# PeterFWS/Structure-PLP-SLAM

Measured on NVIDIA H100. Metric: frames_per_sec_extract_match_poseopt, higher is better.
Workload: dtype u8/f64

## Files before the change

### structure-plp-slam_b200/csrc/orb.cu

```cuda
#include "common.cuh"
#include <cuda.h>
#include <stdlib.h>
#include "brief_pattern.inc"

namespace plp {

namespace {

constexpr int kMaxLevels = 16;
constexpr int kPatchRadius = 19;
constexpr int kHalfPatch = 15;
constexpr int kCellSize = 64;
constexpr int kOverlap = 6;
constexpr int kCellCap = 1024;

struct LevelInfo {
    int w, h, pitch;
    size_t offset;
    size_t blur_offset;
    int cells_x, cells_y;
    int cell_base;
    int num_cells;
    int budget;
    int slot_base;
    int slot_cap;
    float scale_factor;
    float size;
};

struct CellDesc {
    short level, i, j, pad;
    short min_x, min_y, max_x, max_y;
};

struct BlurTile {
    short level, x0, y0, pad;
};

struct LevelKp {
    short x, y;
    int response;
};

struct OrbDev {
    int num_levels, rows, cols;
    int num_cells;
    int total_slots;
    int out_cap;
    int ini_thr, min_thr;
    LevelInfo lv[kMaxLevels];
    int u_max[16];
    const uint8_t *img0;
    size_t img0_step, img0_frame_stride;
    const uint8_t *mask;
    size_t mask_step;
    uint8_t *pyr;
    size_t pyr_frame_bytes;
    uint8_t *blur;
    size_t blur_frame_bytes;
    const BlurTile *blur_tiles;
    int num_blur_tiles;
    const CellDesc *cells;
    uint32_t *cell_buf;
    int *cell_cnt;
    LevelKp *lvl_kp;
    int *lvl_cnt;
    uint8_t *qt_scratch;
    size_t qt_scratch_per_job;
    int *status;
};

__device__ __forceinline__ const uint8_t *level_ptr(const OrbDev &P, int b, int l) {
    return l == 0 ? P.img0 + (size_t)b * P.img0_frame_stride : P.pyr + (size_t)b * P.pyr_frame_bytes + P.lv[l].offset;
}
__device__ __forceinline__ int level_pitch(const OrbDev &P, int l) { return l == 0 ? (int)P.img0_step : P.lv[l].pitch; }

constexpr int kBtW = 64, kBtH = 32;
constexpr int kBoxW = 96, kBoxH = kBtH + 6, kBoxX = 16;
static_assert(kBoxW >= kBoxX + kBtW + 3 && kBoxW % 16 == 0 && kBoxX % 16 == 0 && kBtW % 16 == 0,
              "TMA box: 16-byte aligned start and extent covering the 3-pixel halo");
static_assert(kBoxH % 2 == 0 && kBtH % 2 == 0, "the blur passes work on pairs of rows");
constexpr int kBoxStage = (kBoxH * kBoxW + 127) & ~127;
constexpr int kTilePitch = kBoxW;
constexpr int kTileRows = kCellSize + kOverlap;

struct BlurMaps {
    CUtensorMap m[kMaxLevels];
};

__device__ __forceinline__ uint32_t smem_u32(const void *p) { return (uint32_t)__cvta_generic_to_shared(p); }

__device__ __forceinline__ void mbar_init(uint32_t bar) { asm volatile("mbarrier.init.shared::cta.b64 [%0], 1;" ::"r"(bar)); }

__device__ __forceinline__ bool mbar_wait(uint32_t bar, uint32_t parity) {
    uint32_t done = 0;
    for (int spin = 0; spin < (1 << 14) && !done; ++spin)
        asm volatile(
            "{\n\t.reg .pred p;\n\tmbarrier.try_wait.parity.shared::cta.b64 p, [%1], %2;\n\tselp.u32 %0, 1, 0, p;\n\t}"
            : "=r"(done)
            : "r"(bar), "r"(parity)
            : "memory");
    return done != 0;
}

__device__ __forceinline__ void mbar_expect_tx(uint32_t bar, uint32_t bytes) {
    asm volatile("mbarrier.arrive.expect_tx.shared::cta.b64 _, [%0], %1;" ::"r"(bar), "r"(bytes) : "memory");
}

__device__ __forceinline__ void tma_box_load(uint32_t dst, const CUtensorMap *tm, int x, int y, int f, uint32_t bar) {
    asm volatile(
        "cp.async.bulk.tensor.3d.shared::cluster.global.mbarrier::complete_tx::bytes [%0], [%1, {%2, %3, %4}], [%5];"
        ::"r"(dst), "l"(tm), "r"(x), "r"(y), "r"(f), "r"(bar)
        : "memory");
}

constexpr int kResizeRows = 8;
__global__ void __launch_bounds__(256) pyr_resize_kernel(OrbDev P, int l, const short4 *__restrict__ xtab,
                                                         const short4 *__restrict__ ytab) {
    const int b = blockIdx.y;
    const int dw = P.lv[l].w, dh = P.lv[l].h, dpitch = P.lv[l].pitch;
    const int quads = (dw + 3) >> 2, strips = (dh + kResizeRows - 1) / kResizeRows;
    const int q = blockIdx.x * blockDim.x + threadIdx.x;
    if (q >= quads * strips) return;
    const int strip = q / quads, x0 = (q - strip * quads) * 4;
    const uint8_t *src = level_ptr(P, b, l - 1);
    const int spitch = level_pitch(P, l - 1);
    uint8_t *dst = const_cast<uint8_t *>(level_ptr(P, b, l));
    int sx0[4], sx1[4], a0[4], a1[4];
#pragma unroll
    for (int k = 0; k < 4; ++k) {
        const short4 xt = xtab[min(x0 + k, dw - 1)];
        sx0[k] = xt.x;
        sx1[k] = xt.y;
        a0[k] = xt.z;
        a1[k] = xt.w;
    }
    const int y_end = min(dh, (strip + 1) * kResizeRows);
    for (int y = strip * kResizeRows; y < y_end; ++y) {
        const short4 yt = ytab[y];
        const uint8_t *S0 = src + (size_t)yt.x * spitch, *S1 = src + (size_t)yt.y * spitch;
        const int b0 = yt.z, b1 = yt.w;
        uint32_t packed = 0;
#pragma unroll
        for (int k = 0; k < 4; ++k) {
            const int r0 = S0[sx0[k]] * a0[k] + S0[sx1[k]] * a1[k];
            const int r1 = S1[sx0[k]] * a0[k] + S1[sx1[k]] * a1[k];
            const int v = (((b0 * (r0 >> 4)) >> 16) + ((b1 * (r1 >> 4)) >> 16) + 2) >> 2;
            packed |= (uint32_t)(v & 0xff) << (8 * k);
        }
        *reinterpret_cast<uint32_t *>(dst + (size_t)y * dpitch + x0) = packed;
    }
}

__device__ __forceinline__ uint32_t fast_m_pair(const uint8_t *pa, const uint8_t *pb) {
    const uint32_t v2 = ((uint32_t)pa[0] + 256u) | (((uint32_t)pb[0] + 256u) << 16);
    uint32_t d[16];
#define PLP_RING(k, off) d[k] = v2 - ((uint32_t)pa[off] | ((uint32_t)pb[off] << 16))
    PLP_RING(0, 3 * kTilePitch);
    PLP_RING(1, 3 * kTilePitch + 1);
    PLP_RING(2, 2 * kTilePitch + 2);
    PLP_RING(3, 1 * kTilePitch + 3);
    PLP_RING(4, 3);
    PLP_RING(5, -1 * kTilePitch + 3);
    PLP_RING(6, -2 * kTilePitch + 2);
    PLP_RING(7, -3 * kTilePitch + 1);
    PLP_RING(8, -3 * kTilePitch);
    PLP_RING(9, -3 * kTilePitch - 1);
    PLP_RING(10, -2 * kTilePitch - 2);
    PLP_RING(11, -1 * kTilePitch - 3);
    PLP_RING(12, -3);
    PLP_RING(13, 1 * kTilePitch - 3);
    PLP_RING(14, 2 * kTilePitch - 2);
    PLP_RING(15, 3 * kTilePitch - 1);
#undef PLP_RING
    uint32_t e[16], d2[16], e2[16], d4[16], e4[16];
#pragma unroll
    for (int k = 0; k < 16; ++k) e[k] = 0x02000200u - d[k];
#pragma unroll
    for (int k = 0; k < 16; ++k) {
        d2[k] = __vimin3_s16x2(d[k], d[(k + 1) & 15], d[(k + 1) & 15]);
        e2[k] = __vimin3_s16x2(e[k], e[(k + 1) & 15], e[(k + 1) & 15]);
    }
#pragma unroll
    for (int k = 0; k < 16; ++k) {
        d4[k] = __vimin3_s16x2(d2[k], d2[(k + 2) & 15], d2[(k + 2) & 15]);
        e4[k] = __vimin3_s16x2(e2[k], e2[(k + 2) & 15], e2[(k + 2) & 15]);
    }
    uint32_t best = 0u;
#pragma unroll
    for (int k = 0; k < 16; ++k) {
        const uint32_t d9 = __vimin3_s16x2(d4[k], d4[(k + 4) & 15], d[(k + 8) & 15]);
        const uint32_t e9 = __vimin3_s16x2(e4[k], e4[(k + 4) & 15], e[(k + 8) & 15]);
        best = __vimax3_s16x2(best, d9, e9);
    }
    return best;
}

__device__ __forceinline__ bool masked(const OrbDev &P, unsigned y, unsigned x, float scale) {
    return P.mask[(size_t)(int)(y * scale) * P.mask_step + (int)(x * scale)] == 0;
}


constexpr int kTileX = kPatchRadius % 16;
constexpr int kTestX = kTileX + 3;
static_assert(kCellSize % 16 == 0 && kTestX % 4 == 2, "the pretests below form their words for tested x = 2 (mod 4)");
static_assert(kTileX + kCellSize + kOverlap <= kTilePitch, "a cell row fits a tile row");
constexpr int kFastBox2Row = kTileRows - kBoxH;
static_assert(kFastBox2Row > 0 && kFastBox2Row <= kBoxH && (kFastBox2Row * kTilePitch) % 128 == 0,
              "two boxes cover the tile rows; the second lands 128-byte aligned");
constexpr int kFastStage = (kTileRows * kTilePitch + 127) & ~127;
constexpr int kCornerWords = 4;
static_assert(kCornerWords * 32 >= kTilePitch + 32, "corner bitmap row");

#define PLP_TW(y, k) T32[(y) * (kTilePitch / 4) + (k)]

__device__ __forceinline__ uint32_t compass4(const uint32_t *T32, int y, int k, uint32_t t4) {
    const uint32_t c = __funnelshift_r(PLP_TW(y, k), PLP_TW(y, k + 1), 16);
    const uint32_t up = __funnelshift_r(PLP_TW(y - 3, k), PLP_TW(y - 3, k + 1), 16);
    const uint32_t dn = __funnelshift_r(PLP_TW(y + 3, k), PLP_TW(y + 3, k + 1), 16);
    const uint32_t lf = __funnelshift_r(PLP_TW(y, k - 1), PLP_TW(y, k), 24);
    const uint32_t rt = __funnelshift_r(PLP_TW(y, k + 1), PLP_TW(y, k + 2), 8);
    const uint32_t a0 = __vcmpgtu4(__vabsdiffu4(c, dn), t4), a4 = __vcmpgtu4(__vabsdiffu4(c, rt), t4);
    const uint32_t a8 = __vcmpgtu4(__vabsdiffu4(c, up), t4), a12 = __vcmpgtu4(__vabsdiffu4(c, lf), t4);
    const uint32_t sv = (a4 | a12) & (a0 | a8);
    const uint32_t m = sv & 0x01010101u;
    return (m | (m >> 7) | (m >> 14) | (m >> 21)) & 0xfu;
}

__device__ __forceinline__ uint32_t even8_4(const uint32_t *T32, int y, int k, uint32_t k7) {
    const uint32_t c = __funnelshift_r(PLP_TW(y, k), PLP_TW(y, k + 1), 16);
    auto gt = [&](uint32_t ring) -> uint32_t {
        const uint32_t d = __vabsdiffu4(c, ring);
        return (((d & 0x7f7f7f7fu) + k7) | d) & 0x80808080u;
    };
    const uint32_t e0 = gt(__funnelshift_r(PLP_TW(y + 3, k), PLP_TW(y + 3, k + 1), 16));
    const uint32_t e2 = gt(PLP_TW(y + 2, k + 1));
    const uint32_t e4 = gt(__funnelshift_r(PLP_TW(y, k + 1), PLP_TW(y, k + 2), 8));
    const uint32_t e6 = gt(PLP_TW(y - 2, k + 1));
    const uint32_t e8 = gt(__funnelshift_r(PLP_TW(y - 3, k), PLP_TW(y - 3, k + 1), 16));
    const uint32_t e10 = gt(PLP_TW(y - 2, k));
    const uint32_t e12 = gt(__funnelshift_r(PLP_TW(y, k - 1), PLP_TW(y, k), 24));
    const uint32_t e14 = gt(PLP_TW(y + 2, k));
    const uint32_t p0 = e0 & e2, p2 = e2 & e4, p4 = e4 & e6, p6 = e6 & e8, p8 = e8 & e10, p10 = e10 & e12, p12 = e12 & e14,
                   p14 = e14 & e0;
    const uint32_t r = (p0 & p4) | (p2 & p6) | (p4 & p8) | (p6 & p10) | (p8 & p12) | (p10 & p14) | (p12 & p0) | (p14 & p2);
    return ((r >> 7) | (r >> 14) | (r >> 21) | (r >> 28)) & 0xfu;
}
#undef PLP_TW

struct FastSmem {
    uint8_t score[kTileRows * kTilePitch];
    unsigned corner[kTileRows * kCornerWords];
    unsigned short list[kCellSize * kCellSize];
    unsigned rowbits[128];
    int rowbase[128];
    int wsum[4];
    int nsurv;
};

__device__ __forceinline__ void fast_smem_clear(FastSmem &S) {
    for (int i = threadIdx.x; i < kTileRows * kCornerWords; i += blockDim.x) S.corner[i] = 0u;
    if (threadIdx.x < 128) S.rowbits[threadIdx.x] = 0u;
    if (threadIdx.x == 0) S.nsurv = 0;
}

__device__ __forceinline__ void fast_cell_detect(const OrbDev &P, int ci, const uint8_t *tile, FastSmem &S) {
    const int tid = threadIdx.x, lane = tid & 31, warp = tid >> 5;
    const CellDesc cell = P.cells[ci];
    const int w = cell.max_x - cell.min_x, h = cell.max_y - cell.min_y;
    const float scale = P.lv[cell.level].scale_factor;
    bool skip = (w < 7 || h < 7);
    if (!skip && P.mask) {
        skip = masked(P, cell.min_y, cell.min_x, scale) || masked(P, cell.max_y, cell.min_x, scale) ||
               masked(P, cell.min_y, cell.max_x, scale) || masked(P, cell.max_y, cell.max_x, scale);
    }
    const int tw = w - 6, th = h - 6;
    const uint32_t *T32 = reinterpret_cast<const uint32_t *>(tile);
    for (int pass = 0; !skip; ++pass) {
        const int thr = pass == 0 ? P.ini_thr : P.min_thr;
        const uint32_t t4 = (uint32_t)min(thr, 255) * 0x01010101u;
        const bool strong = thr < 128;
        const uint32_t k7 = (uint32_t)(0x7f - min(thr, 127)) * 0x01010101u;
        for (int rp = warp; rp < (th + 1) / 2; rp += 8) {
            const int ry = 2 * rp + (lane >> 4), g = lane & 15;
            const int nv = tw - 4 * g;
            if (ry >= th || nv <= 0) continue;
            const int y = 3 + ry, k = (kTestX >> 2) + g;
            uint32_t nib = (strong ? even8_4(T32, y, k, k7) : compass4(T32, y, k, t4)) & (nv >= 4 ? 0xfu : (1u << nv) - 1u);
            if (!nib) continue;
            int pos = atomicAdd(&S.nsurv, __popc(nib));
            const int p0 = (y << 7) + kTestX + 4 * g;
            while (nib) {
                const int bit = __ffs(nib) - 1;
                nib &= nib - 1;
                S.list[pos++] = (unsigned short)(p0 + bit);
            }
        }
        __syncthreads();
        const int nsurv = S.nsurv;
        {
            const int half = (nsurv + 1) >> 1;
            for (int i = tid; i < half; i += 256) {
                const int pa = S.list[i];
                const bool has_b = i + half < nsurv;
                const int pb = has_b ? S.list[i + half] : pa;
                const int off_a = (pa >> 7) * kTilePitch + (pa & 127), off_b = (pb >> 7) * kTilePitch + (pb & 127);
                const uint32_t m2 = fast_m_pair(tile + off_a, tile + off_b);
                const int m_a = (int)(m2 & 0xffffu) - 256, m_b = (int)(m2 >> 16) - 256;
                if (m_a > thr) {
                    S.score[off_a] = (uint8_t)(m_a - 1);
                    atomicOr(&S.corner[(pa >> 7) * kCornerWords + ((pa & 127) >> 5)], 1u << (pa & 31));
                }
                if (has_b && m_b > thr) {
                    S.score[off_b] = (uint8_t)(m_b - 1);
                    atomicOr(&S.corner[(pb >> 7) * kCornerWords + ((pb & 127) >> 5)], 1u << (pb & 31));
                }
            }
        }
        __syncthreads();
        bool any_local = false;
        for (int i = tid; i < nsurv; i += 256) {
            const int p = S.list[i];
            const int y = p >> 7, x = p & 127;
            uint32_t nb[3];
#pragma unroll
            for (int r = 0; r < 3; ++r) {
                const unsigned *row = S.corner + (y - 1 + r) * kCornerWords + ((x - 1) >> 5);
                nb[r] = __funnelshift_r(row[0], row[1], (x - 1) & 31) & 7u;
            }
            if (!(nb[1] & 2u)) continue;
            const uint8_t *sp = S.score + y * kTilePitch + x;
            const int sc = sp[0];
            bool keep = true;
#pragma unroll
            for (int dy = -1; dy <= 1; ++dy)
#pragma unroll
                for (int dx = -1; dx <= 1; ++dx) {
                    if (dx == 0 && dy == 0) continue;
                    if (nb[dy + 1] & (1u << (dx + 1))) keep = keep && (sc > (int)sp[dy * kTilePitch + dx]);
                }
            if (keep) {
                const int xx = x - kTestX;
                atomicOr(&S.rowbits[(y - 3) * 2 + (xx >> 5)], 1u << (xx & 31));
                any_local = true;
            }
        }
        const int any = __syncthreads_or(any_local);
        for (int i = tid; i < kTileRows * kCornerWords; i += 256) S.corner[i] = 0u;
        if (tid == 0) S.nsurv = 0;
        if (any || pass == 1 || P.min_thr == P.ini_thr) break;
        __syncthreads();
    }
    if (skip) __syncthreads();
    if (tid < 128) {
        unsigned bits = S.rowbits[tid];
        if (P.mask && bits) {
            unsigned keepbits = bits;
            while (bits) {
                const int bit = __ffs(bits) - 1;
                bits &= bits - 1;
                const int x = 3 + (tid & 1) * 32 + bit, y = 3 + (tid >> 1);
                const float kx = (float)x + (float)(cell.j * kCellSize), ky = (float)y + (float)(cell.i * kCellSize);
                if (masked(P, (unsigned)((float)kPatchRadius + ky), (unsigned)((float)kPatchRadius + kx), scale))
                    keepbits &= ~(1u << bit);
            }
            S.rowbits[tid] = bits = keepbits;
        }
        const int c = __popc(bits);
        int incl = c;
#pragma unroll
        for (int o = 1; o < 32; o <<= 1) {
            const int v = __shfl_up_sync(0xffffffffu, incl, o);
            if (lane >= o) incl += v;
        }
        S.rowbase[tid] = incl - c;
        if (lane == 31) S.wsum[warp] = incl;
    }
}

__device__ __forceinline__ void fast_cell_emit(const OrbDev &P, int b, int ci, FastSmem &S) {
    const int tid = threadIdx.x;
    const CellDesc cell = P.cells[ci];
    if (tid < 128) {
        uint32_t *buf = P.cell_buf + ((size_t)b * P.num_cells + ci) * kCellCap;
        unsigned bits = S.rowbits[tid];
        S.rowbits[tid] = 0u;
        int pos = S.rowbase[tid];
        for (int k = 0; k < (tid >> 5); ++k) pos += S.wsum[k];
        while (bits) {
            const int bit = __ffs(bits) - 1;
            bits &= bits - 1;
            const int x = 3 + (tid & 1) * 32 + bit, y = 3 + (tid >> 1);
            const int sc = S.score[y * kTilePitch + x + kTileX];
            const int lx = x + cell.j * kCellSize, ly = y + cell.i * kCellSize;
            if (pos < kCellCap) buf[pos] = (uint32_t)lx | ((uint32_t)ly << 11) | ((uint32_t)sc << 21);
            ++pos;
        }
    }
    if (tid == 0) P.cell_cnt[(size_t)b * P.num_cells + ci] = min(S.wsum[0] + S.wsum[1] + S.wsum[2] + S.wsum[3], kCellCap);
}

__global__ void __launch_bounds__(256, 4) fast_cells_kernel_v2(OrbDev P) {
    __shared__ __align__(16) uint8_t tile[kTileRows * kTilePitch];
    __shared__ FastSmem S;
    const int b = blockIdx.y, ci = blockIdx.x, tid = threadIdx.x;
    const CellDesc cell = P.cells[ci];
    const int w = cell.max_x - cell.min_x, h = cell.max_y - cell.min_y;
    const uint8_t *img = level_ptr(P, b, cell.level);
    const int pitch = level_pitch(P, cell.level);
    if ((((uintptr_t)img | (uintptr_t)pitch) & 15) == 0) {
        const int nchunks = (kTileX + w + 15) >> 4;
        for (int idx = tid; idx < h * nchunks; idx += 256) {
            const int y = idx / nchunks, c = idx - y * nchunks;
            const uint4 v = __ldg(reinterpret_cast<const uint4 *>(img + (size_t)(cell.min_y + y) * pitch + (cell.min_x - kTileX)) + c);
            *reinterpret_cast<uint4 *>(tile + y * kTilePitch + 16 * c) = v;
        }
    } else {
        for (int y = tid >> 5; y < h; y += 8) {
            const uint8_t *src = img + (size_t)(cell.min_y + y) * pitch + cell.min_x;
            for (int x = tid & 31; x < w; x += 32) tile[y * kTilePitch + kTileX + x] = src[x];
        }
    }
    fast_smem_clear(S);
    __syncthreads();
    fast_cell_detect(P, ci, tile, S);
    __syncthreads();
    fast_cell_emit(P, b, ci, S);
}

constexpr int kFastRun = 4;
__global__ void __launch_bounds__(256, 4) fast_cells_tma_kernel(const __grid_constant__ BlurMaps M, OrbDev P, int run) {
    __shared__ __align__(128) uint8_t s_tile[2][kFastStage];
    __shared__ FastSmem S;
    __shared__ __align__(8) unsigned long long s_bar[2];
    const int b = blockIdx.y, tid = threadIdx.x;
    const int first = blockIdx.x * run, n = min(run, P.num_cells - first);
    if (tid == 0) {
        mbar_init(smem_u32(&s_bar[0]));
        mbar_init(smem_u32(&s_bar[1]));
        asm volatile("fence.mbarrier_init.release.cluster;" ::: "memory");
    }
    fast_smem_clear(S);
    __syncthreads();
    auto issue = [&](int i) {
        const CellDesc c = P.cells[first + i];
        const uint32_t bar = smem_u32(&s_bar[i & 1]), dst = smem_u32(s_tile[i & 1]);
        const CUtensorMap *tm = &M.m[c.level];
        mbar_expect_tx(bar, 2 * kBoxH * kBoxW);
        tma_box_load(dst, tm, c.min_x - kTileX, c.min_y, b, bar);
        tma_box_load(dst + kFastBox2Row * kTilePitch, tm, c.min_x - kTileX, c.min_y + kFastBox2Row, b, bar);
    };
    if (tid == 0) issue(0);
    for (int i = 0; i < n; ++i) {
        __syncthreads();
        if (tid == 0 && i + 1 < n) {
            asm volatile("fence.proxy.async.shared::cta;" ::: "memory");
            issue(i + 1);
        }
        if (i > 0) fast_cell_emit(P, b, first + i - 1, S);
        if (!mbar_wait(smem_u32(&s_bar[i & 1]), (i >> 1) & 1)) P.status[b] = 3;
        fast_cell_detect(P, first + i, s_tile[i & 1], S);
    }
    __syncthreads();
    if (n > 0) fast_cell_emit(P, b, first + n - 1, S);
}

constexpr int kQtThreads = 512;
constexpr int kNodeCap = 2048;
constexpr int kNodeCapSmall = 1024, kCandCapSmall = 3840, kCandCapLarge = 8192;

struct QtArrays {
    uint32_t *cand;
    unsigned short *perm[2];
    unsigned short *owner[2];
};

struct QtNodes {
    short4 *rect;
    unsigned short *start;
    unsigned short *cnt;
    uint8_t *leaf;
};

__device__ __forceinline__ int cand_x(uint32_t c) { return (int)(c & 0x7ff); }
__device__ __forceinline__ int cand_y(uint32_t c) { return (int)((c >> 11) & 0x3ff); }
__device__ __forceinline__ int cand_score(uint32_t c) { return (int)(c >> 21); }

__device__ __forceinline__ int block_exclusive_scan(int v, int *smem_warp , int *total) {
    const int lane = threadIdx.x & 31, warp = threadIdx.x >> 5;
    int incl = v;
#pragma unroll
    for (int o = 1; o < 32; o <<= 1) {
        const int t = __shfl_up_sync(0xffffffffu, incl, o);
        if (lane >= o) incl += t;
    }
    __syncthreads();
    if (lane == 31) smem_warp[warp] = incl;
    __syncthreads();
    if (warp == 0) {
        int s = lane < (kQtThreads / 32) ? smem_warp[lane] : 0;
        int si = s;
#pragma unroll
        for (int o = 1; o < 32; o <<= 1) {
            const int t = __shfl_up_sync(0xffffffffu, si, o);
            if (lane >= o) si += t;
        }
        if (lane < (kQtThreads / 32)) smem_warp[lane] = si - s;
        if (lane == (kQtThreads / 32) - 1) smem_warp[16] = si;
    }
    __syncthreads();
    *total = smem_warp[16];
    return smem_warp[warp] + incl - v;
}

__device__ int block_scan_array(int *data, int n, int *smem_warp) {
    const int per = (n + kQtThreads - 1) / kQtThreads;
    const int i0 = min(n, (int)threadIdx.x * per), i1 = min(n, i0 + per);
    int sum = 0;
    for (int i = i0; i < i1; ++i) sum += data[i];
    int total;
    int run = block_exclusive_scan(sum, smem_warp, &total);
    for (int i = i0; i < i1; ++i) {
        const int v = data[i];
        data[i] = run;
        run += v;
    }
    __syncthreads();
    return total;
}

__device__ __forceinline__ int classify(const short4 r, uint32_t c) {
    const unsigned half_x = (unsigned)cv_ceil((r.z - r.x) / 2.0);
    const unsigned half_y = (unsigned)cv_ceil((r.w - r.y) / 2.0);
    int q = 0;
    if ((float)((unsigned)r.x + half_x) <= (float)cand_x(c)) q += 1;
    if ((float)((unsigned)r.y + half_y) <= (float)cand_y(c)) q += 2;
    return q;
}

__device__ __forceinline__ short4 child_rect(const short4 r, int q) {
    const int half_x = cv_ceil((r.z - r.x) / 2.0), half_y = cv_ceil((r.w - r.y) / 2.0);
    short4 c;
    c.x = (q & 1) ? (short)(r.x + half_x) : r.x;
    c.z = (q & 1) ? r.z : (short)(r.x + half_x);
    c.y = (q & 2) ? (short)(r.y + half_y) : r.y;
    c.w = (q & 2) ? r.w : (short)(r.y + half_y);
    return c;
}

__device__ void segmented_class_scan(const QtArrays &A, int cur, int n, const QtNodes &N, const uint8_t *sel,
                                     unsigned short *rank, uint8_t *cls, unsigned short *tot,
                                     unsigned long long *carry_tail, uint8_t *carry_head) {
    const int tid = threadIdx.x;
    const int per = (n + kQtThreads - 1) / kQtThreads;
    const int i0 = min(n, tid * per), i1 = min(n, i0 + per);
    const unsigned short *perm = A.perm[cur], *owner = A.owner[cur];
    unsigned long long acc = 0;
    bool head = false;
    int prev_owner = (i0 > 0 && i0 < n) ? owner[i0 - 1] : -1;
    for (int i = i0; i < i1; ++i) {
        const int o = owner[i];
        if (o != prev_owner) {
            head = true;
            acc = 0;
        }
        prev_owner = o;
        int q = 0;
        if (sel[o]) q = classify(N.rect[o], A.cand[perm[i]]);
        cls[i] = (uint8_t)q;
        if (sel[o]) acc += 1ull << (16 * q);
    }
    carry_tail[tid] = acc;
    carry_head[tid] = head ? 1 : 0;
    __syncthreads();
    if (tid < 32) {
        constexpr int kPer = kQtThreads / 32;
        unsigned long long run = 0;
        bool hf = false;
        for (int t = tid * kPer; t < (tid + 1) * kPer; ++t) {
            const bool h = carry_head[t] != 0;
            run = h ? carry_tail[t] : run + carry_tail[t];
            hf = hf || h;
        }
        unsigned long long v = run;
        int f = hf ? 1 : 0;
#pragma unroll
        for (int o = 1; o < 32; o <<= 1) {
            const unsigned long long pv = __shfl_up_sync(0xffffffffu, v, o);
            const int pf = __shfl_up_sync(0xffffffffu, f, o);
            if (tid >= o) {
                if (!f) v += pv;
                f |= pf;
            }
        }
        unsigned long long carry = __shfl_up_sync(0xffffffffu, v, 1);
        if (tid == 0) carry = 0;
        run = carry;
        for (int t = tid * kPer; t < (tid + 1) * kPer; ++t) {
            const bool h = carry_head[t] != 0;
            const unsigned long long tail = carry_tail[t];
            carry_tail[t] = run;
            run = h ? tail : run + tail;
        }
    }
    __syncthreads();
    acc = carry_tail[tid];
    prev_owner = (i0 > 0 && i0 < n) ? owner[i0 - 1] : -1;
    for (int i = i0; i < i1; ++i) {
        const int o = owner[i];
        if (o != prev_owner) acc = 0;
        prev_owner = o;
        const int q = cls[i];
        if (sel[o]) {
            rank[i] = (unsigned short)((acc >> (16 * q)) & 0xffff);
            acc += 1ull << (16 * q);
        }
        const bool last = (i + 1 == n) || (owner[i + 1] != o);
        if (last && sel[o]) {
            tot[o * 4 + 0] = (unsigned short)(acc & 0xffff);
            tot[o * 4 + 1] = (unsigned short)((acc >> 16) & 0xffff);
            tot[o * 4 + 2] = (unsigned short)((acc >> 32) & 0xffff);
            tot[o * 4 + 3] = (unsigned short)((acc >> 48) & 0xffff);
        }
    }
    __syncthreads();
}

template <int NC>
struct QtSharedT {
    short4 rect[2][NC];
    unsigned short start[2][NC];
    unsigned short cnt[2][NC];
    uint8_t leaf[2][NC];
    uint8_t sel[NC];
    unsigned short tot[NC * 4];
    int newpos[NC];
    int scan[NC];
    unsigned short pool[2][NC];
    unsigned short pool_sorted[NC];
    unsigned long long carry_tail[kQtThreads];
    uint8_t carry_head[kQtThreads];
    int warp_tmp[17];
    int misc[8];
};

template <int NC>
__device__ int apply_division(QtSharedT<NC> &S, QtArrays &A, int &cur, int n_cand, int &cur_n, int len, int num_proc,
                              const unsigned short *proc_list ,
                              unsigned short *rank, uint8_t *cls, int *pool_len_out, int pool_dst) {
    const int tid = threadIdx.x;
    const int nxt_n = cur_n ^ 1;
    for (int k = tid; k < num_proc; k += kQtThreads) {
        const int p = proc_list[k];
        const unsigned short *t = S.tot + p * 4;
        S.scan[k] = (t[0] > 0) + (t[1] > 0) + (t[2] > 0) + (t[3] > 0);
    }
    __syncthreads();
    const int total_children = block_scan_array(S.scan, num_proc, S.warp_tmp);
    for (int p = tid; p < len; p += kQtThreads) S.newpos[p] = S.sel[p] ? 0 : 1;
    __syncthreads();
    {
    }
    const int kept = block_scan_array(S.newpos, len, S.warp_tmp);
    const int new_len = total_children + kept;
    for (int p = tid; p < len; p += kQtThreads) {
        if (!S.sel[p]) {
            const int pos = total_children + S.newpos[p];
            S.rect[nxt_n][pos] = S.rect[cur_n][p];
            S.start[nxt_n][pos] = S.start[cur_n][p];
            S.cnt[nxt_n][pos] = S.cnt[cur_n][p];
            S.leaf[nxt_n][pos] = S.leaf[cur_n][p];
            S.newpos[p] = pos;
        }
    }
    __syncthreads();
    for (int k = tid; k < num_proc; k += kQtThreads) {
        const int p = proc_list[k];
        const unsigned short *t = S.tot + p * 4;
        const int nch = (t[0] > 0) + (t[1] > 0) + (t[2] > 0) + (t[3] > 0);
        const int base = total_children - S.scan[k] - nch;
        const short4 r = S.rect[cur_n][p];
        int o = S.start[cur_n][p];
        int rnk = 0;
        for (int q = 0; q < 4; ++q) {
            if (t[q] == 0) continue;
            const int pos = base + (nch - 1 - rnk);
            S.rect[nxt_n][pos] = child_rect(r, q);
            S.start[nxt_n][pos] = (unsigned short)o;
            S.cnt[nxt_n][pos] = t[q];
            S.leaf[nxt_n][pos] = 0;
            o += t[q];
            ++rnk;
        }
        S.newpos[p] = base;
    }
    __syncthreads();
    {
        const unsigned short *perm = A.perm[cur], *owner = A.owner[cur];
        unsigned short *perm2 = A.perm[cur ^ 1], *owner2 = A.owner[cur ^ 1];
        for (int i = tid; i < n_cand; i += kQtThreads) {
            const int o = owner[i];
            if (S.sel[o]) {
                const unsigned short *t = S.tot + o * 4;
                const int q = cls[i];
                int off = 0, rnk = 0;
                for (int c = 0; c < q; ++c) {
                    off += t[c];
                    rnk += (t[c] > 0);
                }
                const int nch = (t[0] > 0) + (t[1] > 0) + (t[2] > 0) + (t[3] > 0);
                const int dst = S.start[cur_n][o] + off + rank[i];
                perm2[dst] = perm[i];
                owner2[dst] = (unsigned short)(S.newpos[o] + (nch - 1 - rnk));
            } else {
                perm2[i] = perm[i];
                owner2[i] = (unsigned short)S.newpos[o];
            }
        }
    }
    __syncthreads();
    for (int k = tid; k < num_proc; k += kQtThreads) {
        const unsigned short *t = S.tot + proc_list[k] * 4;
        S.scan[k] = (t[0] > 1) + (t[1] > 1) + (t[2] > 1) + (t[3] > 1);
    }
    __syncthreads();
    const int pool_len = block_scan_array(S.scan, num_proc, S.warp_tmp);
    for (int k = tid; k < num_proc; k += kQtThreads) {
        const int p = proc_list[k];
        const unsigned short *t = S.tot + p * 4;
        const int nch = (t[0] > 0) + (t[1] > 0) + (t[2] > 0) + (t[3] > 0);
        int w = S.scan[k], rnk = 0;
        for (int q = 0; q < 4; ++q) {
            if (t[q] == 0) continue;
            if (t[q] > 1) S.pool[pool_dst][w++] = (unsigned short)(S.newpos[p] + (nch - 1 - rnk));
            ++rnk;
        }
    }
    __syncthreads();
    *pool_len_out = pool_len;
    cur ^= 1;
    cur_n = nxt_n;
    return new_len;
}

template <int NC, int CC, int kMinBlocks>
__global__ void __launch_bounds__(kQtThreads, kMinBlocks) quadtree_kernel(OrbDev P) {
    extern __shared__ __align__(16) uint8_t qsmem[];
    using QtShared = QtSharedT<NC>;
    constexpr int kQtSmemCands = CC;
    QtShared &S = *reinterpret_cast<QtShared *>(qsmem);
    const int l = blockIdx.x, b = blockIdx.y, tid = threadIdx.x;
    const LevelInfo &LV = P.lv[l];
    int *lvl_cnt = P.lvl_cnt + (size_t)b * P.num_levels + l;
    LevelKp *out = P.lvl_kp + (size_t)b * P.total_slots + LV.slot_base;

    const int *cc = P.cell_cnt + (size_t)b * P.num_cells + LV.cell_base;
    for (int c = tid; c < LV.num_cells; c += kQtThreads) S.scan[c] = cc[c];
    __syncthreads();
    int n = block_scan_array(S.scan, LV.num_cells, S.warp_tmp);
    if (n == 0) {
        if (tid == 0) *lvl_cnt = 0;
        return;
    }
    if (n > 65535) {
        n = 65535;
        if (tid == 0) P.status[b] = 1;
    }
    QtArrays A;
    unsigned short *rank;
    uint8_t *cls;
    {
        uint8_t *base;
        if (n <= kQtSmemCands) {
            base = qsmem + ((sizeof(QtShared) + 15) & ~(size_t)15);
        } else {
            base = P.qt_scratch + ((size_t)b * P.num_levels + l) * P.qt_scratch_per_job;
        }
        const size_t cap = n <= kQtSmemCands ? kQtSmemCands : 65536;
        A.cand = reinterpret_cast<uint32_t *>(base);
        base += cap * 4;
        A.perm[0] = reinterpret_cast<unsigned short *>(base);
        base += cap * 2;
        A.perm[1] = reinterpret_cast<unsigned short *>(base);
        base += cap * 2;
        A.owner[0] = reinterpret_cast<unsigned short *>(base);
        base += cap * 2;
        A.owner[1] = reinterpret_cast<unsigned short *>(base);
        base += cap * 2;
        rank = reinterpret_cast<unsigned short *>(base);
        base += cap * 2;
        cls = base;
    }
    {
        const uint32_t *cb = P.cell_buf + ((size_t)b * P.num_cells + LV.cell_base) * kCellCap;
        for (int c = 0; c < LV.num_cells; ++c) {
            const int o = S.scan[c], k = cc[c];
            for (int i = tid; i < k; i += kQtThreads)
                if (o + i < n) A.cand[o + i] = cb[(size_t)c * kCellCap + i];
        }
    }
    __syncthreads();

    const int min_x = kPatchRadius, max_x = LV.w - kPatchRadius, min_y = kPatchRadius, max_y = LV.h - kPatchRadius;
    const double ratio = (double)(max_x - min_x) / (max_y - min_y);
    int gx, gy;
    double dx, dy;
    if (ratio > 1) {
        gx = (int)round(ratio);
        gy = 1;
        dx = (double)(max_x - min_x) / gx;
        dy = max_y - min_y;
    } else {
        gx = 1;
        gy = (int)round(1 / ratio);
        dx = max_x - min_y;
        dy = (double)(max_y - min_y) / gy;
    }
    const int g = gx * gy;
    int cur = 0, cur_n = 0, len = 0;
    {
        int *cnts = S.scan;
        for (int i = tid; i < g; i += kQtThreads) cnts[i] = 0;
        __syncthreads();
        for (int i = tid; i < n; i += kQtThreads) {
            const uint32_t c = A.cand[i];
            const unsigned ix = (unsigned)((float)cand_x(c) / dx), iy = (unsigned)((float)cand_y(c) / dy);
            int node = (int)(ix + iy * gx);
            node = min(node, g - 1);
            cls[i] = 0;
            A.owner[0][i] = (unsigned short)node;
            atomicAdd(&cnts[node], 1);
        }
        __syncthreads();
        if (tid == 0) {
            int off = 0, pos = 0;
            for (int i = 0; i < g; ++i) {
                const int c = cnts[i];
                S.newpos[i] = off;
                if (c > 0) {
                    const int ix = i % gx, iy = i / gx;
                    short4 r;
                    r.x = (short)(int)(dx * ix);
                    r.y = (short)(int)(dy * iy);
                    r.z = (short)(int)(dx * (ix + 1));
                    r.w = (short)(int)(dy * (iy + 1));
                    S.rect[0][pos] = r;
                    S.start[0][pos] = (unsigned short)off;
                    S.cnt[0][pos] = (unsigned short)c;
                    S.leaf[0][pos] = (c == 1);
                    S.tot[i] = (unsigned short)pos;
                    ++pos;
                }
                off += c;
            }
            S.misc[0] = pos;
        }
        __syncthreads();
        len = S.misc[0];
        for (int node = 0; node < g; ++node) {
            if (cnts[node] == 0) continue;
            const int per = (n + kQtThreads - 1) / kQtThreads;
            const int i0 = min(n, tid * per), i1 = min(n, i0 + per);
            int c = 0;
            for (int i = i0; i < i1; ++i) c += (A.owner[0][i] == node);
            int tot;
            int run = block_exclusive_scan(c, S.warp_tmp, &tot);
            const int base = S.newpos[node];
            const unsigned short lp = S.tot[node];
            for (int i = i0; i < i1; ++i)
                if (A.owner[0][i] == node) {
                    A.perm[1][base + run] = (unsigned short)i;
                    A.owner[1][base + run] = lp;
                    ++run;
                }
            __syncthreads();
        }
        cur = 1;
    }
    const int budget = LV.budget;
    int pool_len = 0, pool_cur = 0;
    bool filled = false;
    unsigned short *proc_list = S.pool_sorted;

    while (true) {
        const int prev = len;
        for (int p = tid; p < len; p += kQtThreads) S.sel[p] = S.leaf[cur_n][p] ? 0 : 1;
        __syncthreads();
        for (int p = tid; p < len; p += kQtThreads) S.scan[p] = S.sel[p];
        __syncthreads();
        const int num_proc = block_scan_array(S.scan, len, S.warp_tmp);
        for (int p = tid; p < len; p += kQtThreads)
            if (S.sel[p]) proc_list[S.scan[p]] = (unsigned short)p;
        __syncthreads();
        segmented_class_scan(A, cur, n, QtNodes{S.rect[cur_n], S.start[cur_n], S.cnt[cur_n], S.leaf[cur_n]}, S.sel,
                             rank, cls, S.tot, S.carry_tail, S.carry_head);
        len = apply_division(S, A, cur, n, cur_n, len, num_proc, proc_list, rank, cls, &pool_len, pool_cur);
        if (budget <= len || len == prev) {
            filled = true;
            break;
        }
        if (budget < len + pool_len) break;
    }
    while (!filled) {
        const int prev = len;
        const unsigned short *pool = S.pool[pool_cur];
        for (int p = tid; p < len; p += kQtThreads) S.sel[p] = 0;
        __syncthreads();
        for (int k = tid; k < pool_len; k += kQtThreads) S.sel[pool[k]] = 1;
        __syncthreads();
        segmented_class_scan(A, cur, n, QtNodes{S.rect[cur_n], S.start[cur_n], S.cnt[cur_n], S.leaf[cur_n]}, S.sel,
                             rank, cls, S.tot, S.carry_tail, S.carry_head);
        for (int k = tid; k < pool_len; k += kQtThreads) {
            const int ck = S.cnt[cur_n][pool[k]];
            int r = 0;
            for (int j = 0; j < pool_len; ++j) {
                const int cj = S.cnt[cur_n][pool[j]];
                r += (cj > ck) || (cj == ck && j > k);
            }
            proc_list[r] = pool[k];
        }
        __syncthreads();
        for (int k = tid; k < pool_len; k += kQtThreads) {
            const unsigned short *t = S.tot + proc_list[k] * 4;
            S.scan[k] = (t[0] > 0) + (t[1] > 0) + (t[2] > 0) + (t[3] > 0) - 1;
        }
        if (tid == 0) {
            S.misc[1] = pool_len;
            S.misc[2] = 0;
        }
        __syncthreads();
        block_scan_array(S.scan, pool_len, S.warp_tmp);
        for (int k = tid; k < pool_len; k += kQtThreads) {
            const unsigned short *t = S.tot + proc_list[k] * 4;
            const int inc = (t[0] > 0) + (t[1] > 0) + (t[2] > 0) + (t[3] > 0) - 1;
            if (prev + S.scan[k] + inc >= budget) {
                atomicMin(&S.misc[1], k + 1);
                S.misc[2] = 1;
            }
        }
        __syncthreads();
        const int num_proc = S.misc[1];
        const bool reached = S.misc[2] != 0;
        __syncthreads();
        for (int k = num_proc + tid; k < pool_len; k += kQtThreads) S.sel[proc_list[k]] = 0;
        __syncthreads();
        len = apply_division(S, A, cur, n, cur_n, len, num_proc, proc_list, rank, cls, &pool_len, pool_cur ^ 1);
        pool_cur ^= 1;
        if (reached) filled = true;
        if (filled || budget <= len || len == prev) break;
    }

    const int n_out = min(len, LV.slot_cap);
    if (len > LV.slot_cap && tid == 0) P.status[b] = 3;
    for (int p = tid; p < n_out; p += kQtThreads) {
        const int st = S.start[cur_n][p], c = S.cnt[cur_n][p];
        uint32_t best = A.cand[A.perm[cur][st]];
        for (int k = 1; k < c; ++k) {
            const uint32_t v = A.cand[A.perm[cur][st + k]];
            if (cand_score(v) > cand_score(best)) best = v;
        }
        LevelKp kp;
        kp.x = (short)(cand_x(best) + kPatchRadius);
        kp.y = (short)(cand_y(best) + kPatchRadius);
        kp.response = cand_score(best);
        out[p] = kp;
    }
    if (tid == 0) *lvl_cnt = n_out;
}

constexpr int kDescWarps = 4;
constexpr int kDescRun = 8;
constexpr int kDescMinBlocks = 5;
constexpr int kDiscRows = 2 * kHalfPatch + 1, kDiscPitch = 48;
constexpr int kWinHalf = 18, kWinRows = 2 * kWinHalf + 1, kWinPitch = 64;
constexpr int kDiscBytes = kDiscRows * kDiscPitch;
constexpr int kDescStage = kDiscBytes + kWinRows * kWinPitch;
static_assert(kDiscBytes % 16 == 0 && kDescStage % 16 == 0, "16-byte copies into every row of the ring");
static_assert(15 + kDiscRows <= kDiscPitch && 15 + kWinRows <= kWinPitch, "the aligned supersets fit the rows");

__device__ __forceinline__ int reflect101(int p, int len) {
    if (p < 0) p = -p;
    if (p >= len) p = 2 * (len - 1) - p;
    return p;
}

__device__ __forceinline__ float fast_atan2_deg(float y, float x) {
    const float scale = (float)(180.0 / 3.14159265358979323846);
    const float p1 = 0.9997878412794807f * scale, p3 = -0.3258083974640975f * scale,
                p5 = 0.1555786518463281f * scale, p7 = -0.04432655554792128f * scale;
    const float ax = fabsf(x), ay = fabsf(y);
    float a, c, c2;
    if (ax >= ay) {
        c = __fdiv_rn(ay, ax + (float)2.2204460492503131e-16);
        c2 = c * c;
        a = (((p7 * c2 + p5) * c2 + p3) * c2 + p1) * c;
    } else {
        c = __fdiv_rn(ax, ay + (float)2.2204460492503131e-16);
        c2 = c * c;
        a = 90.f - (((p7 * c2 + p5) * c2 + p3) * c2 + p1) * c;
    }
    if (x < 0) a = 180.f - a;
    if (y < 0) a = 360.f - a;
    return a;
}

__device__ __forceinline__ float poly_cos(float v) {
    const float c1 = 0.99940307f, c2 = -0.49558072f, c3 = 0.03679168f;
    const float v2 = v * v;
    return c1 + v2 * (c2 + c3 * v2);
}
__device__ __forceinline__ float util_cos(float v) {
    const float PI = 3.14159265358979f, PI_2 = PI / 2.0f, TWO_PI = 2.0f * PI, INV_TWO_PI = 1.0f / TWO_PI,
                THREE_PI_2 = 3.0f * PI_2;
    v = v - (float)cv_floor((double)(v * INV_TWO_PI)) * TWO_PI;
    v = (0.0f < v) ? v : -v;
    if (v < PI_2) return poly_cos(v);
    if (v < PI) return -poly_cos(PI - v);
    if (v < THREE_PI_2) return -poly_cos(v - PI);
    return poly_cos(TWO_PI - v);
}
__device__ __forceinline__ float util_sin(float v) {
    const float PI_2 = 3.14159265358979f / 2.0f;
    return util_cos(PI_2 - v);
}


__device__ __forceinline__ void blur_row4(const uint32_t *w, uint32_t h[4]) {
    const uint32_t A = w[0], B = w[1], C = w[2];
    const uint32_t kW1 = 0x38302212u, kW2 = 0x00122230u;
    h[0] = __dp4a(__funnelshift_r(A, B, 8), kW1, __dp4a(__funnelshift_r(B, C, 8), kW2, 0u));
    h[1] = __dp4a(__funnelshift_r(A, B, 16), kW1, __dp4a(__funnelshift_r(B, C, 16), kW2, 0u));
    h[2] = __dp4a(__funnelshift_r(A, B, 24), kW1, __dp4a(__funnelshift_r(B, C, 24), kW2, 0u));
    h[3] = __dp4a(B, kW1, __dp4a(C, kW2, 0u));
}
__device__ __forceinline__ void blur_h_pass(const uint8_t *box, uint32_t *h2) {
    const uint32_t *src32 = reinterpret_cast<const uint32_t *>(box);
    for (int i = threadIdx.x; i < (kBoxH / 2) * (kBtW / 4); i += blockDim.x) {
        const int rp = i / (kBtW / 4), j = i % (kBtW / 4);
        const uint32_t *w = src32 + 2 * rp * (kBoxW / 4) + j + (kBoxX - 4) / 4;
        uint32_t e[4], o[4];
        blur_row4(w, e);
        blur_row4(w + kBoxW / 4, o);
        *reinterpret_cast<uint4 *>(h2 + rp * kBtW + 4 * j) =
            make_uint4(__byte_perm(e[0], o[0], 0x5410), __byte_perm(e[1], o[1], 0x5410), __byte_perm(e[2], o[2], 0x5410),
                       __byte_perm(e[3], o[3], 0x5410));
    }
}

constexpr int kBlurThreads = 256;
static_assert((kBtH / 2) * (kBtW / 4) == kBlurThreads, "one vertical-pass job per thread");
__device__ __forceinline__ void blur_v_pass(const uint32_t *h2, uint8_t *dst, int dpitch, int x0, int y0, int W, int H) {
    const int q = threadIdx.x / (kBtW / 4), px = (threadIdx.x % (kBtW / 4)) * 4;
    const int y = y0 + 2 * q;
    if (y >= H || x0 + px >= W) return;
    uint32_t r[4][4];
#pragma unroll
    for (int k = 0; k < 4; ++k) {
        const uint4 v = *reinterpret_cast<const uint4 *>(h2 + (q + k) * kBtW + px);
        r[k][0] = v.x;
        r[k][1] = v.y;
        r[k][2] = v.z;
        r[k][3] = v.w;
    }
    auto row = [&](uint32_t k0, uint32_t k1, uint32_t k2, uint32_t k3) -> uint32_t {
        uint32_t a[4];
#pragma unroll
        for (int c = 0; c < 4; ++c)
            a[c] = __dp2a_lo(r[0][c], k0, __dp2a_lo(r[1][c], k1, __dp2a_lo(r[2][c], k2, __dp2a_lo(r[3][c], k3, 32768u))));
        return __byte_perm(__byte_perm(a[0], a[1], 0x0062), __byte_perm(a[2], a[3], 0x0062), 0x5410);
    };
    uint8_t *d = dst + (size_t)y * dpitch + x0 + px;
    *reinterpret_cast<uint32_t *>(d) = row(0x2212u, 0x3830u, 0x2230u, 0x0012u);
    if (y + 1 < H) *reinterpret_cast<uint32_t *>(d + dpitch) = row(0x1200u, 0x3022u, 0x3038u, 0x1222u);
}

__global__ void __launch_bounds__(kBlurThreads) blur_tiles_kernel(OrbDev P) {
    __shared__ __align__(16) uint8_t s_src[kBoxH * kBoxW];
    __shared__ __align__(16) uint32_t s_h2[(kBoxH / 2) * kBtW];
    const int b = blockIdx.y, tid = threadIdx.x;
    const BlurTile t = P.blur_tiles[blockIdx.x];
    const int l = t.level, W = P.lv[l].w, H = P.lv[l].h;
    const uint8_t *img = level_ptr(P, b, l);
    const int pitch = level_pitch(P, l);
    constexpr int kCols = kBtW + 8;
    for (int i = tid; i < kBoxH * kCols; i += kBlurThreads) {
        const int py = i / kCols, px = i - py * kCols;
        const int gy = reflect101(min(t.y0 - 3 + py, H + 2), H);
        const int gx = reflect101(min(max(t.x0 - 4 + px, -3), W + 2), W);
        s_src[py * kBoxW + kBoxX - 4 + px] = img[(size_t)gy * pitch + gx];
    }
    __syncthreads();
    blur_h_pass(s_src, s_h2);
    __syncthreads();
    blur_v_pass(s_h2, P.blur + (size_t)b * P.blur_frame_bytes + P.lv[l].blur_offset, P.lv[l].pitch, t.x0, t.y0, W, H);
}

__device__ void blur_reflect_box(uint8_t *box, int bx0, int by0, int W, int H) {
    for (int i = threadIdx.x; i < kBoxH * 6; i += blockDim.x) {
        const int py = i / 6, k = i - py * 6;
        const int gx = k < 3 ? k - 3 : W + (k - 3), gy = by0 + py;
        const int px = gx - bx0;
        if (gy < 0 || gy >= H || px < 0 || px >= kBoxW) continue;
        box[py * kBoxW + px] = box[py * kBoxW + (reflect101(gx, W) - bx0)];
    }
    __syncthreads();
    for (int i = threadIdx.x; i < 6 * kBoxW; i += blockDim.x) {
        const int k = i / kBoxW, px = i - k * kBoxW;
        const int gy = k < 3 ? k - 3 : H + (k - 3);
        const int py = gy - by0;
        if (py < 0 || py >= kBoxH) continue;
        box[py * kBoxW + px] = box[(reflect101(gy, H) - by0) * kBoxW + px];
    }
    __syncthreads();
}

constexpr int kBlurRun = 4;
__global__ void __launch_bounds__(kBlurThreads) blur_tiles_tma_kernel(const __grid_constant__ BlurMaps M, OrbDev P, int run) {
    __shared__ __align__(128) uint8_t s_src[2][kBoxStage];
    __shared__ __align__(16) uint32_t s_h2[(kBoxH / 2) * kBtW];
    __shared__ __align__(8) unsigned long long s_bar[2];
    const int b = blockIdx.y, tid = threadIdx.x;
    const int first = blockIdx.x * run, n = min(run, P.num_blur_tiles - first);
    if (tid == 0) {
        mbar_init(smem_u32(&s_bar[0]));
        mbar_init(smem_u32(&s_bar[1]));
        asm volatile("fence.mbarrier_init.release.cluster;" ::: "memory");
    }
    __syncthreads();
    auto issue = [&](int i) {
        const BlurTile t = P.blur_tiles[first + i];
        const uint32_t bar = smem_u32(&s_bar[i & 1]);
        mbar_expect_tx(bar, kBoxH * kBoxW);
        tma_box_load(smem_u32(s_src[i & 1]), &M.m[t.level], t.x0 - kBoxX, t.y0 - 3, b, bar);
    };
    if (tid == 0) issue(0);
    for (int i = 0; i < n; ++i) {
        __syncthreads();
        if (tid == 0 && i + 1 < n) {
            asm volatile("fence.proxy.async.shared::cta;" ::: "memory");
            issue(i + 1);
        }
        const BlurTile t = P.blur_tiles[first + i];
        const int l = t.level, W = P.lv[l].w, H = P.lv[l].h;
        const int bx0 = t.x0 - kBoxX, by0 = t.y0 - 3;
        uint8_t *box = s_src[i & 1];
        if (!mbar_wait(smem_u32(&s_bar[i & 1]), (i >> 1) & 1)) P.status[b] = 3;
        if (t.x0 < 3 || by0 < 0 || t.x0 + kBtW + 3 > W || by0 + kBoxH > H) blur_reflect_box(box, bx0, by0, W, H);
        blur_h_pass(box, s_h2);
        __syncthreads();
        blur_v_pass(s_h2, P.blur + (size_t)b * P.blur_frame_bytes + P.lv[l].blur_offset, P.lv[l].pitch, t.x0, t.y0, W, H);
    }
}

__device__ __forceinline__ void cp_async16(void *dst, const void *src) {
    asm volatile("cp.async.ca.shared.global [%0], [%1], 16;" ::"r"(smem_u32(dst)), "l"(src) : "memory");
}
__device__ __forceinline__ void cp_async_commit() { asm volatile("cp.async.commit_group;" ::: "memory"); }
__device__ __forceinline__ void cp_async_wait_prev() { asm volatile("cp.async.wait_group 1;" ::: "memory"); }

__device__ __forceinline__ int dp4a_us(uint32_t a, uint32_t b, int c) {
    int d;
    asm("dp4a.u32.s32 %0, %1, %2, %3;" : "=r"(d) : "r"(a), "r"(b), "r"(c));
    return d;
}

template <int J>
__device__ __forceinline__ void disc_row_sums(const uint32_t (&r)[12], int sh, const uint32_t (&wu)[8],
                                              const uint32_t (&wm)[8], int &su, int &si) {
#pragma unroll
    for (int k = 0; k < 8; ++k) {
        const uint32_t w = __funnelshift_r(r[J + k], r[J + k + 1], sh);
        su = dp4a_us(w, wu[k], su);
        si = dp4a_us(w, wm[k], si);
    }
}

__global__ void __launch_bounds__(kDescWarps * 32, kDescMinBlocks) describe_kernel(OrbDev P, plp_keypoint *__restrict__ kp_out,
                                                                    uint8_t *__restrict__ desc_out,
                                                                    int32_t *__restrict__ n_out) {
    __shared__ __align__(16) uint8_t s_ring[kDescWarps][2][kDescStage];
    __shared__ int s_cum[kMaxLevels + 1];
    __shared__ const uint8_t *s_img[kMaxLevels], *s_blur[kMaxLevels];
    __shared__ int s_pitch[kMaxLevels], s_bpitch[kMaxLevels], s_slot[kMaxLevels];
    __shared__ float s_scale[kMaxLevels], s_size[kMaxLevels];
    const int b = blockIdx.y, warp = threadIdx.x >> 5, lane = threadIdx.x & 31;
    if (warp == 0) {
        const int l = lane;
        int c = l < P.num_levels ? P.lvl_cnt[(size_t)b * P.num_levels + l] : 0;
#pragma unroll
        for (int o = 1; o < 32; o <<= 1) {
            const int t = __shfl_up_sync(0xffffffffu, c, o);
            if (lane >= o) c += t;
        }
        if (l == 0) s_cum[0] = 0;
        if (l < kMaxLevels) s_cum[l + 1] = c;
        if (l < P.num_levels) {
            s_img[l] = level_ptr(P, b, l);
            s_pitch[l] = level_pitch(P, l);
            s_blur[l] = P.blur + (size_t)b * P.blur_frame_bytes + P.lv[l].blur_offset;
            s_bpitch[l] = P.lv[l].pitch;
            s_slot[l] = P.lv[l].slot_base;
            s_scale[l] = P.lv[l].scale_factor;
            s_size[l] = P.lv[l].size;
        }
    }
    const bool vec0 = ((reinterpret_cast<uintptr_t>(P.img0) | P.img0_step | P.img0_frame_stride) & 15) == 0;
    uint32_t wu[8], wm[8];
    {
        const int dv = lane - kHalfPatch, umax = lane < kDiscRows ? P.u_max[dv < 0 ? -dv : dv] : -1;
#pragma unroll
        for (int k = 0; k < 8; ++k) {
            wu[k] = wm[k] = 0;
#pragma unroll
            for (int c = 0; c < 4; ++c) {
                const int u = 4 * k + c - kHalfPatch;
                if (u <= kHalfPatch && (u < 0 ? -u : u) <= umax) {
                    wu[k] |= (uint32_t)(u & 0xff) << (8 * c);
                    wm[k] |= 1u << (8 * c);
                }
            }
        }
    }
    float x1[8], y1[8], x2[8], y2[8];
    {
        const uint2 px1 = __ldg(reinterpret_cast<const uint2 *>(kBriefX1) + lane), py1 = __ldg(reinterpret_cast<const uint2 *>(kBriefY1) + lane);
        const uint2 px2 = __ldg(reinterpret_cast<const uint2 *>(kBriefX2) + lane), py2 = __ldg(reinterpret_cast<const uint2 *>(kBriefY2) + lane);
#pragma unroll
        for (int bit = 0; bit < 8; ++bit) {
            const int sh = (bit & 3) * 8;
            x1[bit] = (float)(signed char)(((bit < 4 ? px1.x : px1.y) >> sh) & 0xff);
            y1[bit] = (float)(signed char)(((bit < 4 ? py1.x : py1.y) >> sh) & 0xff);
            x2[bit] = (float)(signed char)(((bit < 4 ? px2.x : px2.y) >> sh) & 0xff);
            y2[bit] = (float)(signed char)(((bit < 4 ? py2.x : py2.y) >> sh) & 0xff);
        }
    }
    __syncthreads();
    const int total = min(s_cum[kMaxLevels], P.out_cap);
    if (blockIdx.x == 0 && threadIdx.x == 0) n_out[b] = total;
    const LevelKp *frame_kp = P.lvl_kp + (size_t)b * P.total_slots;
    uint8_t(*ring)[kDescStage] = s_ring[warp];
    for (int p0 = (blockIdx.x * kDescWarps + warp) * kDescRun; p0 < total; p0 += gridDim.x * kDescWarps * kDescRun) {
        const int n = min(kDescRun, total - p0);
        int ml = 0, mx = 0, my = 0, mresp = 0;
        if (lane < n) {
            const int pos = p0 + lane;
            while (pos >= s_cum[ml + 1]) ++ml;
            const LevelKp kp = frame_kp[s_slot[ml] + pos - s_cum[ml]];
            mx = kp.x;
            my = kp.y;
            mresp = kp.response;
        }
        auto stage = [&](int i) {
            const int cx = __shfl_sync(0xffffffffu, mx, i), cy = __shfl_sync(0xffffffffu, my, i),
                      l = __shfl_sync(0xffffffffu, ml, i);
            uint8_t *disc = ring[i & 1], *win = disc + kDiscBytes;
            const int xw = cx - kWinHalf, ow = xw & 15, nw = (ow + kWinRows + 15) >> 4, bpitch = s_bpitch[l];
            const uint8_t *bsrc = s_blur[l] + (size_t)(cy - kWinHalf) * bpitch + (xw - ow);
#pragma unroll
            for (int t = lane; t < kWinRows * 4; t += 32) {
                const int r = t >> 2, c = t & 3;
                if (c < nw) cp_async16(win + r * kWinPitch + 16 * c, bsrc + (size_t)r * bpitch + 16 * c);
            }
            const int xd = cx - kHalfPatch, od = xd & 15, pitch = s_pitch[l];
            const uint8_t *dsrc = s_img[l] + (size_t)(cy - kHalfPatch) * pitch;
            if (l > 0 || vec0) {
                const int nd = (od + kDiscRows + 15) >> 4;
                dsrc += xd - od;
#pragma unroll
                for (int t = lane; t < kDiscRows * 3; t += 32) {
                    const int r = t / 3, c = t - 3 * r;
                    if (c < nd) cp_async16(disc + r * kDiscPitch + 16 * c, dsrc + (size_t)r * pitch + 16 * c);
                }
            } else if (lane < kDiscRows) {
#pragma unroll 8
                for (int r = 0; r < kDiscRows; ++r)
                    disc[r * kDiscPitch + od + lane] = __ldg(dsrc + (size_t)r * pitch + xd + lane);
            }
        };
        stage(0);
        cp_async_commit();
        float my_angle = 0.f;
        for (int i = 0; i < n; ++i) {
            if (i + 1 < n) stage(i + 1);
            cp_async_commit();
            cp_async_wait_prev();
            __syncwarp();
            const int cx = __shfl_sync(0xffffffffu, mx, i);
            const uint8_t *disc = ring[i & 1], *win = disc + kDiscBytes;

            int su = 0, si = 0;
            {
                const uint4 *row = reinterpret_cast<const uint4 *>(disc + min(lane, kDiscRows - 1) * kDiscPitch);
                const uint4 q0 = row[0], q1 = row[1], q2 = row[2];
                const uint32_t r[12] = {q0.x, q0.y, q0.z, q0.w, q1.x, q1.y, q1.z, q1.w, q2.x, q2.y, q2.z, q2.w};
                const int od = (cx - kHalfPatch) & 15, sh = 8 * (od & 3);
                switch (od >> 2) {
                    case 0: disc_row_sums<0>(r, sh, wu, wm, su, si); break;
                    case 1: disc_row_sums<1>(r, sh, wu, wm, su, si); break;
                    case 2: disc_row_sums<2>(r, sh, wu, wm, su, si); break;
                    default: disc_row_sums<3>(r, sh, wu, wm, su, si); break;
                }
            }
            int m10 = su, m01 = (lane - kHalfPatch) * si;
#pragma unroll
            for (int o = 16; o > 0; o >>= 1) {
                m10 += __shfl_xor_sync(0xffffffffu, m10, o);
                m01 += __shfl_xor_sync(0xffffffffu, m01, o);
            }
            const float angle = fast_atan2_deg((float)m01, (float)m10);

            const float ang_rad = (float)((double)angle * 3.14159265358979323846 / 180.0);
            const float ca = util_cos(ang_rad), sa = util_sin(ang_rad);
            const uint8_t *center = win + kWinHalf * kWinPitch + kWinHalf + ((cx - kWinHalf) & 15);
            int val = 0;
#pragma unroll
            for (int bit = 0; bit < 8; ++bit) {
                const int r1 = __float2int_rn(x1[bit] * sa + y1[bit] * ca), c1 = __float2int_rn(x1[bit] * ca - y1[bit] * sa);
                const int r2 = __float2int_rn(x2[bit] * sa + y2[bit] * ca), c2 = __float2int_rn(x2[bit] * ca - y2[bit] * sa);
                val |= (center[r1 * kWinPitch + c1] < center[r2 * kWinPitch + c2]) << bit;
            }
            desc_out[((size_t)b * P.out_cap + p0 + i) * 32 + lane] = (uint8_t)val;
            if (lane == i) my_angle = angle;
            __syncwarp();
        }
        if (lane < n) {
            plp_keypoint o;
            const float s = s_scale[ml];
            o.x = ml == 0 ? (float)mx : (float)mx * s;
            o.y = ml == 0 ? (float)my : (float)my * s;
            o.size = s_size[ml];
            o.angle = my_angle;
            o.response = (float)mresp;
            o.octave = ml;
            o.class_id = -1;
            kp_out[(size_t)b * P.out_cap + p0 + lane] = o;
        }
    }
}

}

}

using namespace plp;

struct plp_orb {
    plp_ctx *ctx = nullptr;
    plp_orb_params params;
    int rows = 0, cols = 0, max_batch = 0;
    OrbDev dev;
    std::vector<float> scale_factors, inv_scale_factors, level_sigma_sq, inv_level_sigma_sq;
    std::vector<uint32_t> num_keypts_per_level;
    std::vector<CellDesc> cells;
    short4 *d_xtab[kMaxLevels] = {nullptr};
    short4 *d_ytab[kMaxLevels] = {nullptr};
    CellDesc *d_cells = nullptr;
    uint8_t *d_pyr = nullptr;
    uint8_t *d_blur = nullptr;
    BlurTile *d_blur_tiles = nullptr;
    std::vector<BlurTile> blur_tiles;
    uint8_t *d_img = nullptr;
    uint8_t *d_mask = nullptr;
    uint32_t *d_cell_buf = nullptr;
    int *d_cell_cnt = nullptr;
    LevelKp *d_lvl_kp = nullptr;
    int *d_lvl_cnt = nullptr;
    uint8_t *d_qt_scratch = nullptr;
    int *d_status = nullptr;
    plp_keypoint *d_kp = nullptr;
    uint8_t *d_desc = nullptr;
    int32_t *d_n = nullptr;
    size_t qt_smem = 0;
    bool qt_small = false;
    BlurMaps maps;
    bool maps_ok = false;
    const uint8_t *map0_img = nullptr;
    size_t map0_step = 0;
    int map0_batch = 0;
    int last_batch = 0;
    const uint8_t *last_img0 = nullptr;
    size_t last_step = 0;
};

typedef CUresult (*EncodeTiledFn)(CUtensorMap *, CUtensorMapDataType, cuuint32_t, void *, const cuuint64_t *, const cuuint64_t *,
                                  const cuuint32_t *, const cuuint32_t *, CUtensorMapInterleave, CUtensorMapSwizzle,
                                  CUtensorMapL2promotion, CUtensorMapFloatOOBfill);
static EncodeTiledFn tensor_map_encoder() {
    static EncodeTiledFn fn = []() -> EncodeTiledFn {
        void *p = nullptr;
        cudaDriverEntryPointQueryResult q;
        if (cudaGetDriverEntryPoint("cuTensorMapEncodeTiled", &p, cudaEnableDefault, &q) != cudaSuccess ||
            q != cudaDriverEntryPointSuccess)
            return nullptr;
        return (EncodeTiledFn)p;
    }();
    return fn;
}
static bool encode_level_map(CUtensorMap *m, const uint8_t *base, int w, int h, int frames, size_t pitch, size_t frame_stride) {
    EncodeTiledFn enc = tensor_map_encoder();
    if (!enc || ((uintptr_t)base & 15) || (pitch & 15) || (frame_stride & 15) || w < 1 || h < 1 || frames < 1) return false;
    const cuuint64_t dims[3] = {(cuuint64_t)w, (cuuint64_t)h, (cuuint64_t)frames};
    const cuuint64_t strides[2] = {(cuuint64_t)pitch, (cuuint64_t)frame_stride};
    const cuuint32_t box[3] = {(cuuint32_t)kBoxW, (cuuint32_t)kBoxH, 1u}, estr[3] = {1u, 1u, 1u};
    return enc(m, CU_TENSOR_MAP_DATA_TYPE_UINT8, 3, (void *)base, dims, strides, box, estr, CU_TENSOR_MAP_INTERLEAVE_NONE,
               CU_TENSOR_MAP_SWIZZLE_NONE, CU_TENSOR_MAP_L2_PROMOTION_L2_128B, CU_TENSOR_MAP_FLOAT_OOB_FILL_NONE) == CUDA_SUCCESS;
}


static void build_resize_tables(int sw, int sh, int dw, int dh, std::vector<short4> &xt, std::vector<short4> &yt) {
    const double inv_scale_x = (double)dw / sw, inv_scale_y = (double)dh / sh;
    const double scale_x = 1. / inv_scale_x, scale_y = 1. / inv_scale_y;
    xt.resize(dw);
    yt.resize(dh);
    for (int dx = 0; dx < dw; ++dx) {
        float fx = (float)((dx + 0.5) * scale_x - 0.5);
        int sx = cv_floor(fx);
        fx -= sx;
        if (sx < 0) {
            fx = 0;
            sx = 0;
        }
        if (sx >= sw - 1) {
            fx = 0;
            sx = sw - 1;
        }
        short4 t;
        t.x = (short)sx;
        t.y = (short)std::min(sx + 1, sw - 1);
        t.z = (short)lrintf((1.f - fx) * 2048);
        t.w = (short)lrintf(fx * 2048);
        xt[dx] = t;
    }
    for (int dy = 0; dy < dh; ++dy) {
        float fy = (float)((dy + 0.5) * scale_y - 0.5);
        int sy = cv_floor(fy);
        fy -= sy;
        short4 t;
        t.x = (short)std::min(std::max(sy, 0), sh - 1);
        t.y = (short)std::min(std::max(sy + 1, 0), sh - 1);
        t.z = (short)lrintf((1.f - fy) * 2048);
        t.w = (short)lrintf(fy * 2048);
        yt[dy] = t;
    }
}

extern "C" {

void plp_orb_destroy(plp_orb *o) {
    if (!o) return;
    cudaSetDevice(o->ctx->device);
    cudaStreamSynchronize(o->ctx->stream);
    for (int l = 0; l < kMaxLevels; ++l) {
        if (o->d_xtab[l]) cudaFree(o->d_xtab[l]);
        if (o->d_ytab[l]) cudaFree(o->d_ytab[l]);
    }
    void *ptrs[] = {o->d_blur, o->d_blur_tiles, o->d_cells, o->d_pyr, o->d_img, o->d_mask, o->d_cell_buf, o->d_cell_cnt, o->d_lvl_kp,
                    o->d_lvl_cnt, o->d_qt_scratch, o->d_status, o->d_kp, o->d_desc, o->d_n};
    for (void *p : ptrs)
        if (p) cudaFree(p);
    delete o;
}

plp_status plp_orb_create(plp_ctx *ctx, const plp_orb_params *params, int rows, int cols, int max_batch,
                          plp_orb **out) {
    PLP_REQUIRE(ctx && params && out, "null pointer");
    *out = nullptr;
    PLP_REQUIRE(rows > 0 && cols > 0 && max_batch > 0, "image size / batch");
    PLP_REQUIRE(params->num_levels >= 1 && params->num_levels <= kMaxLevels, "num_levels in [1,16]");
    PLP_REQUIRE(params->scale_factor > 1.0f || params->num_levels == 1, "scale_factor > 1");
    PLP_REQUIRE(cols <= 2047 + 2 * kPatchRadius && rows <= 1023 + 2 * kPatchRadius,
                "image larger than 2085 x 1061 (packed candidate coordinates)");
    PLP_REQUIRE(params->ini_fast_thr < 255 && params->min_fast_thr >= 1 && params->min_fast_thr <= params->ini_fast_thr,
                "FAST thresholds: 1 <= min <= ini < 255");
    PLP_CUDA_TRY(cudaSetDevice(ctx->device));
    plp_orb *o = new plp_orb();
    o->ctx = ctx;
    o->params = *params;
    o->rows = rows;
    o->cols = cols;
    o->max_batch = max_batch;
    const unsigned L = params->num_levels;
    o->scale_factors.assign(L, 1.0f);
    o->inv_scale_factors.assign(L, 1.0f);
    o->level_sigma_sq.assign(L, 1.0f);
    o->inv_level_sigma_sq.assign(L, 1.0f);
    for (unsigned l = 1; l < L; ++l) o->scale_factors[l] = params->scale_factor * o->scale_factors[l - 1];
    for (unsigned l = 1; l < L; ++l) o->inv_scale_factors[l] = (1.0f / params->scale_factor) * o->inv_scale_factors[l - 1];
    {
        float s = 1.0f;
        for (unsigned l = 1; l < L; ++l) {
            s = params->scale_factor * s;
            o->level_sigma_sq[l] = s * s;
            o->inv_level_sigma_sq[l] = 1.0f / (s * s);
        }
    }
    o->num_keypts_per_level.resize(L);
    {
        double desired = params->max_num_keypts * (1.0 - 1.0 / params->scale_factor) /
                         (1.0 - std::pow(1.0 / params->scale_factor, static_cast<double>(L)));
        if (L == 1) desired = params->max_num_keypts;
        unsigned total = 0;
        for (unsigned l = 0; l + 1 < L; ++l) {
            o->num_keypts_per_level[l] = (unsigned)std::round(desired);
            total += o->num_keypts_per_level[l];
            desired *= 1.0 / params->scale_factor;
        }
        o->num_keypts_per_level[L - 1] = (unsigned)std::max((int)params->max_num_keypts - (int)total, 0);
    }
    OrbDev &D = o->dev;
    memset(&D, 0, sizeof(D));
    D.num_levels = (int)L;
    D.rows = rows;
    D.cols = cols;
    D.ini_thr = (int)params->ini_fast_thr;
    D.min_thr = (int)params->min_fast_thr;
    {
        const unsigned vmax = (unsigned)std::floor(kHalfPatch * std::sqrt(2.0) / 2 + 1);
        const unsigned vmin = (unsigned)std::ceil(kHalfPatch * std::sqrt(2.0) / 2);
        for (unsigned v = 0; v <= vmax; ++v)
            D.u_max[v] = (int)std::round(std::sqrt((double)kHalfPatch * kHalfPatch - (double)v * v));
        for (unsigned v = kHalfPatch, v0 = 0; vmin <= v; --v) {
            while (D.u_max[v0] == D.u_max[v0 + 1]) ++v0;
            D.u_max[v] = (int)v0;
            ++v0;
        }
    }
    int qt_max_slots = 0;
    size_t pyr_bytes = 0, blur_bytes = 0;
    int slot_base = 0, cell_base = 0;
    plp_status st = PLP_OK;
    for (unsigned l = 0; l < L; ++l) {
        LevelInfo &V = D.lv[l];
        if (l == 0) {
            V.w = cols;
            V.h = rows;
        } else {
            const double scale = o->scale_factors[l];
            V.w = (int)std::round(cols * 1.0 / scale);
            V.h = (int)std::round(rows * 1.0 / scale);
        }
        V.pitch = (V.w + 63) & ~63;
        V.offset = pyr_bytes;
        if (l > 0) pyr_bytes += (size_t)V.pitch * V.h + 256;
        pyr_bytes = (pyr_bytes + 255) & ~(size_t)255;
        V.blur_offset = blur_bytes;
        blur_bytes += (size_t)V.pitch * V.h + 256;
        blur_bytes = (blur_bytes + 255) & ~(size_t)255;
        for (int y0 = 0; y0 < V.h; y0 += kBtH)
            for (int x0 = 0; x0 < V.w; x0 += kBtW) o->blur_tiles.push_back(BlurTile{(short)l, (short)x0, (short)y0, 0});
        V.budget = (int)o->num_keypts_per_level[l];
        V.scale_factor = o->scale_factors[l];
        V.size = (float)(unsigned)(31 * o->scale_factors[l]);
        V.slot_base = slot_base;
        {
            int g0 = 1;
            if (V.w > 2 * kPatchRadius && V.h > 2 * kPatchRadius) {
                const double ratio = (double)(V.w - 2 * kPatchRadius) / (V.h - 2 * kPatchRadius);
                g0 = ratio > 1 ? (int)std::round(ratio) : (int)std::round(1 / ratio);
            }
            V.slot_cap = 4 * std::max(V.budget, g0) + 8;
        }
        slot_base += V.slot_cap;
        V.cell_base = cell_base;
        V.num_cells = 0;
        qt_max_slots = std::max(qt_max_slots, V.slot_cap);
        if (V.slot_cap > kNodeCap) {
            set_error("orb: level %u budget %d exceeds the quadtree node capacity", l, V.budget);
            st = PLP_ERR_CAPACITY;
        }
        if (V.w > 2 * kPatchRadius && V.h > 2 * kPatchRadius && V.w >= 1 && V.h >= 1) {
            const unsigned min_bx = kPatchRadius, min_by = kPatchRadius;
            const unsigned max_bx = V.w - kPatchRadius, max_by = V.h - kPatchRadius;
            const unsigned width = max_bx - min_bx, height = max_by - min_by;
            const unsigned ncols = width / kCellSize + 1, nrows = height / kCellSize + 1;
            V.cells_x = (int)ncols;
            V.cells_y = (int)nrows;
            for (unsigned i = 0; i < nrows; ++i) {
                const unsigned min_y = min_by + i * kCellSize;
                if (max_by - kOverlap <= min_y || max_by < kOverlap) continue;
                unsigned max_y = min_y + kCellSize + kOverlap;
                if (max_by < max_y) max_y = max_by;
                for (unsigned j = 0; j < ncols; ++j) {
                    const unsigned min_x = min_bx + j * kCellSize;
                    if (max_bx - kOverlap <= min_x || max_bx < kOverlap) continue;
                    unsigned max_x = min_x + kCellSize + kOverlap;
                    if (max_bx < max_x) max_x = max_bx;
                    CellDesc c;
                    c.level = (short)l;
                    c.i = (short)i;
                    c.j = (short)j;
                    c.pad = 0;
                    c.min_x = (short)min_x;
                    c.min_y = (short)min_y;
                    c.max_x = (short)max_x;
                    c.max_y = (short)max_y;
                    o->cells.push_back(c);
                    V.num_cells++;
                }
            }
        }
        cell_base += V.num_cells;
    }
    if (st != PLP_OK) {
        delete o;
        return st;
    }
    D.num_cells = cell_base;
    D.total_slots = slot_base;
    D.out_cap = slot_base;
    D.pyr_frame_bytes = pyr_bytes ? pyr_bytes : 256;
    D.blur_frame_bytes = blur_bytes ? blur_bytes : 256;
    D.num_blur_tiles = (int)o->blur_tiles.size();
    const size_t B = (size_t)max_batch;
#define ORB_ALLOC(ptr, bytes)                                              \
    do {                                                                   \
        cudaError_t e_ = cudaMalloc((void **)&(ptr), (bytes) ? (bytes) : 256); \
        if (e_ != cudaSuccess) {                                           \
            set_error("orb: cudaMalloc(%zu) failed: %s", (size_t)(bytes), cudaGetErrorString(e_)); \
            plp_orb_destroy(o);                                            \
            return PLP_ERR_CUDA;                                           \
        }                                                                  \
    } while (0)
    for (unsigned l = 1; l < L; ++l) {
        std::vector<short4> xt, yt;
        build_resize_tables(D.lv[l - 1].w, D.lv[l - 1].h, D.lv[l].w, D.lv[l].h, xt, yt);
        ORB_ALLOC(o->d_xtab[l], xt.size() * sizeof(short4));
        ORB_ALLOC(o->d_ytab[l], yt.size() * sizeof(short4));
        cudaMemcpy(o->d_xtab[l], xt.data(), xt.size() * sizeof(short4), cudaMemcpyHostToDevice);
        cudaMemcpy(o->d_ytab[l], yt.data(), yt.size() * sizeof(short4), cudaMemcpyHostToDevice);
    }
    ORB_ALLOC(o->d_cells, o->cells.size() * sizeof(CellDesc));
    if (!o->cells.empty())
        cudaMemcpy(o->d_cells, o->cells.data(), o->cells.size() * sizeof(CellDesc), cudaMemcpyHostToDevice);
    ORB_ALLOC(o->d_pyr, B * D.pyr_frame_bytes);
    ORB_ALLOC(o->d_blur, B * D.blur_frame_bytes);
    ORB_ALLOC(o->d_blur_tiles, o->blur_tiles.size() * sizeof(BlurTile));
    if (!o->blur_tiles.empty())
        cudaMemcpy(o->d_blur_tiles, o->blur_tiles.data(), o->blur_tiles.size() * sizeof(BlurTile), cudaMemcpyHostToDevice);
    ORB_ALLOC(o->d_img, B * (size_t)rows * cols);
    ORB_ALLOC(o->d_mask, (size_t)rows * cols);
    ORB_ALLOC(o->d_cell_buf, B * (size_t)D.num_cells * kCellCap * sizeof(uint32_t));
    ORB_ALLOC(o->d_cell_cnt, B * (size_t)D.num_cells * sizeof(int));
    ORB_ALLOC(o->d_lvl_kp, B * (size_t)D.total_slots * sizeof(LevelKp));
    ORB_ALLOC(o->d_lvl_cnt, B * L * sizeof(int));
    D.qt_scratch_per_job = (size_t)65536 * (4 + 2 * 5 + 1) + 256;
    ORB_ALLOC(o->d_qt_scratch, B * L * D.qt_scratch_per_job);
    ORB_ALLOC(o->d_status, B * sizeof(int));
    ORB_ALLOC(o->d_kp, B * (size_t)D.out_cap * sizeof(plp_keypoint));
    ORB_ALLOC(o->d_desc, B * (size_t)D.out_cap * 32);
    ORB_ALLOC(o->d_n, B * sizeof(int32_t));
#undef ORB_ALLOC
    D.pyr = o->d_pyr;
    D.blur = o->d_blur;
    D.blur_tiles = o->d_blur_tiles;
    D.cells = o->d_cells;
    D.cell_buf = o->d_cell_buf;
    D.cell_cnt = o->d_cell_cnt;
    D.lvl_kp = o->d_lvl_kp;
    D.lvl_cnt = o->d_lvl_cnt;
    D.qt_scratch = o->d_qt_scratch;
    D.status = o->d_status;
    o->maps_ok = true;
    memset(&o->maps, 0, sizeof(o->maps));
    for (unsigned l = 1; l < L && o->maps_ok; ++l)
        o->maps_ok = encode_level_map(&o->maps.m[l], o->d_pyr + D.lv[l].offset, D.lv[l].w, D.lv[l].h, max_batch, D.lv[l].pitch,
                                      D.pyr_frame_bytes);
    o->qt_small = qt_max_slots <= kNodeCapSmall;
    plp_status so;
    if (o->qt_small) {
        o->qt_smem = ((sizeof(QtSharedT<kNodeCapSmall>) + 15) & ~(size_t)15) + (size_t)kCandCapSmall * (4 + 2 * 5 + 1) + 64;
        so = ensure_smem_optin((const void *)quadtree_kernel<kNodeCapSmall, kCandCapSmall, 2>, o->qt_smem, "quadtree_kernel<small>");
    } else {
        o->qt_smem = ((sizeof(QtSharedT<kNodeCap>) + 15) & ~(size_t)15) + (size_t)kCandCapLarge * (4 + 2 * 5 + 1) + 64;
        so = ensure_smem_optin((const void *)quadtree_kernel<kNodeCap, kCandCapLarge, 1>, o->qt_smem, "quadtree_kernel<large>");
    }
    if (so != PLP_OK) {
        plp_orb_destroy(o);
        return so;
    }
    *out = o;
    return PLP_OK;
}

int plp_orb_capacity(const plp_orb *o) { return o ? o->dev.out_cap : 0; }

plp_status plp_orb_get_tables(const plp_orb *o, float *sf, float *isf, float *ls, float *ils, uint32_t *nk) {
    PLP_REQUIRE(o, "orb");
    for (int l = 0; l < o->dev.num_levels; ++l) {
        if (sf) sf[l] = o->scale_factors[l];
        if (isf) isf[l] = o->inv_scale_factors[l];
        if (ls) ls[l] = o->level_sigma_sq[l];
        if (ils) ils[l] = o->inv_level_sigma_sq[l];
        if (nk) nk[l] = o->num_keypts_per_level[l];
    }
    return PLP_OK;
}

static plp_status orb_run(plp_orb *o, const uint8_t *d_imgs, int batch, size_t step, const uint8_t *d_mask,
                          size_t mask_step, plp_keypoint *d_kp, uint8_t *d_desc, int32_t *d_n, int32_t *d_status) {
    plp_ctx *ctx = o->ctx;
    OrbDev D = o->dev;
    D.img0 = d_imgs;
    D.img0_step = step;
    D.img0_frame_stride = step * (size_t)o->rows;
    D.mask = d_mask;
    D.mask_step = mask_step;
    D.status = d_status ? d_status : o->d_status;
    o->last_batch = batch;
    o->last_img0 = d_imgs;
    o->last_step = step;
    PLP_CUDA_TRY(cudaMemsetAsync(D.status, 0, (size_t)batch * sizeof(int), ctx->stream));
    for (int l = 1; l < D.num_levels; ++l) {
        const int quads = ((D.lv[l].w + 3) >> 2) * ((D.lv[l].h + kResizeRows - 1) / kResizeRows);
        if (quads <= 0) continue;
        dim3 grid(div_up(quads, 256), batch);
        PLP_LAUNCH(ctx, pyr_resize_kernel, grid, 256, 0, D, l, o->d_xtab[l], o->d_ytab[l]);
    }
    bool tma = o->maps_ok;
    if (tma && (o->map0_img != d_imgs || o->map0_step != step || o->map0_batch != batch)) {
        tma = encode_level_map(&o->maps.m[0], d_imgs, D.lv[0].w, D.lv[0].h, batch, step, D.img0_frame_stride);
        o->map0_img = tma ? d_imgs : nullptr;
        o->map0_step = step;
        o->map0_batch = batch;
    }
    if (D.num_cells > 0) {
        dim3 grid(D.num_cells, batch), grid_run(div_up(D.num_cells, kFastRun), batch);
        if (tma)
            PLP_LAUNCH(ctx, fast_cells_tma_kernel, grid_run, 256, 0, o->maps, D, kFastRun);
        else
            PLP_LAUNCH(ctx, fast_cells_kernel_v2, grid, 256, 0, D);
    }
    if (D.num_blur_tiles > 0) {
        dim3 grid(D.num_blur_tiles, batch), grid_run(div_up(D.num_blur_tiles, kBlurRun), batch);
        if (tma)
            PLP_LAUNCH(ctx, blur_tiles_tma_kernel, grid_run, kBlurThreads, 0, o->maps, D, kBlurRun);
        else
            PLP_LAUNCH(ctx, blur_tiles_kernel, grid, kBlurThreads, 0, D);
    }
    {
        dim3 grid(D.num_levels, batch);
        if (ctx->timing) plp::timing_begin(ctx, o->qt_small ? "quadtree_kernel<1024>" : "quadtree_kernel<2048>");
        if (o->qt_small)
            quadtree_kernel<kNodeCapSmall, kCandCapSmall, 2><<<grid, kQtThreads, o->qt_smem, ctx->stream>>>(D);
        else
            quadtree_kernel<kNodeCap, kCandCapLarge, 1><<<grid, kQtThreads, o->qt_smem, ctx->stream>>>(D);
        if (ctx->timing) plp::timing_end(ctx);
        ctx->launches++;
    }
    {
        const int kp_est = std::max(256, (int)o->params.max_num_keypts);
        dim3 grid(div_up(std::min(D.total_slots, kp_est), kDescWarps * kDescRun), batch);
        PLP_LAUNCH(ctx, describe_kernel, grid, kDescWarps * 32, 0, D, d_kp, d_desc, d_n);
    }
    PLP_CHECK_LAUNCH();
    return PLP_OK;
}

plp_status plp_orb_extract_batch_dev(plp_orb *o, const uint8_t *d_imgs, int batch, size_t step, plp_keypoint *d_kp,
                                     uint8_t *d_desc, int32_t *d_n, int32_t *d_status) {
    PLP_REQUIRE(o && d_imgs && d_kp && d_desc && d_n, "null pointer");
    PLP_REQUIRE(batch >= 1 && batch <= o->max_batch, "batch exceeds the handle's max_batch");
    PLP_REQUIRE(step >= (size_t)o->cols, "step < cols");
    PLP_CUDA_TRY(cudaSetDevice(o->ctx->device));
    return orb_run(o, d_imgs, batch, step, nullptr, 0, d_kp, d_desc, d_n, d_status);
}

static plp_status orb_extract_host(plp_orb *o, const uint8_t *imgs, int batch, size_t step, const uint8_t *mask,
                                   size_t mask_step, plp_keypoint *kp_out, uint8_t *desc_out, int32_t *n_out) {
    plp_ctx *ctx = o->ctx;
    PLP_CUDA_TRY(cudaSetDevice(ctx->device));
    const size_t rows = o->rows, cols = o->cols;
    PLP_CUDA_TRY(cudaMemcpy2DAsync(o->d_img, cols, imgs, step, cols, rows * (size_t)batch, cudaMemcpyHostToDevice,
                                   ctx->stream));
    const uint8_t *d_mask = nullptr;
    if (mask) {
        PLP_CUDA_TRY(cudaMemcpy2DAsync(o->d_mask, cols, mask, mask_step, cols, rows, cudaMemcpyHostToDevice, ctx->stream));
        d_mask = o->d_mask;
    }
    PLP_TRY(orb_run(o, o->d_img, batch, cols, d_mask, cols, o->d_kp, o->d_desc, o->d_n, nullptr));
    const size_t cap = o->dev.out_cap;
    PLP_CUDA_TRY(cudaMemcpyAsync(n_out, o->d_n, (size_t)batch * 4, cudaMemcpyDeviceToHost, ctx->stream));
    PLP_CUDA_TRY(cudaMemcpyAsync(kp_out, o->d_kp, (size_t)batch * cap * sizeof(plp_keypoint), cudaMemcpyDeviceToHost,
                                 ctx->stream));
    PLP_CUDA_TRY(cudaMemcpyAsync(desc_out, o->d_desc, (size_t)batch * cap * 32, cudaMemcpyDeviceToHost, ctx->stream));
    std::vector<int> status(batch);
    PLP_CUDA_TRY(cudaMemcpyAsync(status.data(), o->d_status, (size_t)batch * 4, cudaMemcpyDeviceToHost, ctx->stream));
    PLP_CUDA_TRY(cudaStreamSynchronize(ctx->stream));
    for (int b = 0; b < batch; ++b)
        if (status[b] != 0) {
            set_error("orb: capacity overflow in frame %d (code %d)", b, status[b]);
            return PLP_ERR_CAPACITY;
        }
    return PLP_OK;
}

plp_status plp_orb_extract(plp_orb *o, const uint8_t *img, int rows, int cols, size_t step, const uint8_t *mask,
                           size_t mask_step, plp_keypoint *kp_out, uint8_t *desc_out, int *n_out) {
    PLP_REQUIRE(o && n_out, "null pointer");
    *n_out = 0;
    if (!img || rows == 0 || cols == 0) return PLP_OK;
    PLP_REQUIRE(rows == o->rows && cols == o->cols, "image size differs from the handle's");
    PLP_REQUIRE(kp_out && desc_out, "null output");
    PLP_REQUIRE(step >= (size_t)cols && (!mask || mask_step >= (size_t)cols), "step < cols");
    int32_t n = 0;
    PLP_TRY(orb_extract_host(o, img, 1, step, mask, mask_step, kp_out, desc_out, &n));
    *n_out = n;
    return PLP_OK;
}

plp_status plp_orb_extract_batch(plp_orb *o, const uint8_t *imgs, int batch, size_t step, plp_keypoint *kp_out,
                                 uint8_t *desc_out, int32_t *n_out) {
    PLP_REQUIRE(o && imgs && kp_out && desc_out && n_out, "null pointer");
    PLP_REQUIRE(batch >= 1 && batch <= o->max_batch, "batch exceeds the handle's max_batch");
    PLP_REQUIRE(step >= (size_t)o->cols, "step < cols");
    return orb_extract_host(o, imgs, batch, step, nullptr, 0, kp_out, desc_out, n_out);
}

plp_status plp_orb_get_pyramid(const plp_orb *o, int b, int level, plp_image_view *out) {
    PLP_REQUIRE(o && out, "null pointer");
    PLP_REQUIRE(b >= 0 && b < o->last_batch && level >= 0 && level < o->dev.num_levels, "index");
    const LevelInfo &V = o->dev.lv[level];
    out->rows = V.h;
    out->cols = V.w;
    if (level == 0) {
        out->data = o->last_img0 + (size_t)b * o->last_step * o->rows;
        out->step = o->last_step;
    } else {
        out->data = o->d_pyr + (size_t)b * o->dev.pyr_frame_bytes + V.offset;
        out->step = V.pitch;
    }
    return PLP_OK;
}

plp_status plp_orb_debug_blurred(plp_orb *o, int b, int level, uint8_t *out) {
    PLP_REQUIRE(o && out, "null pointer");
    PLP_REQUIRE(b >= 0 && b < o->last_batch && level >= 0 && level < o->dev.num_levels, "index");
    plp_ctx *ctx = o->ctx;
    PLP_CUDA_TRY(cudaSetDevice(ctx->device));
    const LevelInfo &V = o->dev.lv[level];
    PLP_CUDA_TRY(cudaStreamSynchronize(ctx->stream));
    PLP_CUDA_TRY(cudaMemcpy2D(out, V.w, o->d_blur + (size_t)b * o->dev.blur_frame_bytes + V.blur_offset, V.pitch, V.w, V.h,
                              cudaMemcpyDeviceToHost));
    return PLP_OK;
}

plp_status plp_orb_debug_candidates(plp_orb *o, int b, int level, plp_keypoint *out, int cap, int *n_out) {
    PLP_REQUIRE(o && out && n_out, "null pointer");
    PLP_REQUIRE(b >= 0 && b < o->last_batch && level >= 0 && level < o->dev.num_levels, "index");
    plp_ctx *ctx = o->ctx;
    PLP_CUDA_TRY(cudaSetDevice(ctx->device));
    const LevelInfo &V = o->dev.lv[level];
    std::vector<int> cnt(V.num_cells);
    std::vector<uint32_t> buf((size_t)V.num_cells * kCellCap);
    PLP_CUDA_TRY(cudaStreamSynchronize(ctx->stream));
    if (V.num_cells) {
        PLP_CUDA_TRY(cudaMemcpy(cnt.data(), o->d_cell_cnt + (size_t)b * o->dev.num_cells + V.cell_base,
                                cnt.size() * 4, cudaMemcpyDeviceToHost));
        PLP_CUDA_TRY(cudaMemcpy(buf.data(), o->d_cell_buf + ((size_t)b * o->dev.num_cells + V.cell_base) * kCellCap,
                                buf.size() * 4, cudaMemcpyDeviceToHost));
    }
    int n = 0;
    for (int c = 0; c < V.num_cells; ++c)
        for (int k = 0; k < cnt[c]; ++k) {
            if (n < cap) {
                const uint32_t v = buf[(size_t)c * kCellCap + k];
                plp_keypoint kp;
                kp.x = (float)(v & 0x7ff);
                kp.y = (float)((v >> 11) & 0x3ff);
                kp.size = 7.f;
                kp.angle = -1.f;
                kp.response = (float)(v >> 21);
                kp.octave = 0;
                kp.class_id = -1;
                out[n] = kp;
            }
            ++n;
        }
    *n_out = n;
    return PLP_OK;
}

}
```

Measured before the change: 83470.

## Move quadtree kernel into a separate header and parallelize candidate gather

Moves the ORB quadtree distribution kernel into its own header with a thread-count template parameter. Candidate gathering now runs in parallel over all candidates, using a binary search on per-cell prefix sums with batched __ldg loads, instead of looping over cells one at a time. The pool-ordering and division steps are restructured: pool nodes are ranked by count in parallel, and the budget cutoff is found with a block scan plus atomicMin. Shared memory uses unions and 16-bit positions, which shrinks the footprint but adds complexity and risks subtle ordering differences.

```diff
diff --git a/structure-plp-slam_b200/csrc/orb.cu b/structure-plp-slam_b200/csrc/orb.cu
--- a/structure-plp-slam_b200/csrc/orb.cu
+++ b/structure-plp-slam_b200/csrc/orb.cu
@@ -2,17 +2,16 @@
 #include <cuda.h>
 #include <stdlib.h>
 #include "brief_pattern.inc"
+#include "quadtree_kernels.cuh"
 
 namespace plp {
 
 namespace {
 
 constexpr int kMaxLevels = 16;
-constexpr int kPatchRadius = 19;
 constexpr int kHalfPatch = 15;
 constexpr int kCellSize = 64;
 constexpr int kOverlap = 6;
-constexpr int kCellCap = 1024;
 
 struct LevelInfo {
     int w, h, pitch;
@@ -35,11 +34,6 @@
 
 struct BlurTile {
     short level, x0, y0, pad;
-};
-
-struct LevelKp {
-    short x, y;
-    int response;
 };
 
 struct OrbDev {
@@ -465,509 +459,6 @@
     if (n > 0) fast_cell_emit(P, b, first + n - 1, S);
 }
 
-constexpr int kQtThreads = 512;
-constexpr int kNodeCap = 2048;
-constexpr int kNodeCapSmall = 1024, kCandCapSmall = 3840, kCandCapLarge = 8192;
-
-struct QtArrays {
-    uint32_t *cand;
-    unsigned short *perm[2];
-    unsigned short *owner[2];
-};
-
-struct QtNodes {
-    short4 *rect;
-    unsigned short *start;
-    unsigned short *cnt;
-    uint8_t *leaf;
-};
-
-__device__ __forceinline__ int cand_x(uint32_t c) { return (int)(c & 0x7ff); }
-__device__ __forceinline__ int cand_y(uint32_t c) { return (int)((c >> 11) & 0x3ff); }
-__device__ __forceinline__ int cand_score(uint32_t c) { return (int)(c >> 21); }
-
-__device__ __forceinline__ int block_exclusive_scan(int v, int *smem_warp , int *total) {
-    const int lane = threadIdx.x & 31, warp = threadIdx.x >> 5;
-    int incl = v;
-#pragma unroll
-    for (int o = 1; o < 32; o <<= 1) {
-        const int t = __shfl_up_sync(0xffffffffu, incl, o);
-        if (lane >= o) incl += t;
-    }
-    __syncthreads();
-    if (lane == 31) smem_warp[warp] = incl;
-    __syncthreads();
-    if (warp == 0) {
-        int s = lane < (kQtThreads / 32) ? smem_warp[lane] : 0;
-        int si = s;
-#pragma unroll
-        for (int o = 1; o < 32; o <<= 1) {
-            const int t = __shfl_up_sync(0xffffffffu, si, o);
-            if (lane >= o) si += t;
-        }
-        if (lane < (kQtThreads / 32)) smem_warp[lane] = si - s;
-        if (lane == (kQtThreads / 32) - 1) smem_warp[16] = si;
-    }
-    __syncthreads();
-    *total = smem_warp[16];
-    return smem_warp[warp] + incl - v;
-}
-
-__device__ int block_scan_array(int *data, int n, int *smem_warp) {
-    const int per = (n + kQtThreads - 1) / kQtThreads;
-    const int i0 = min(n, (int)threadIdx.x * per), i1 = min(n, i0 + per);
-    int sum = 0;
-    for (int i = i0; i < i1; ++i) sum += data[i];
-    int total;
-    int run = block_exclusive_scan(sum, smem_warp, &total);
-    for (int i = i0; i < i1; ++i) {
-        const int v = data[i];
-        data[i] = run;
-        run += v;
-    }
-    __syncthreads();
-    return total;
-}
-
-__device__ __forceinline__ int classify(const short4 r, uint32_t c) {
-    const unsigned half_x = (unsigned)cv_ceil((r.z - r.x) / 2.0);
-    const unsigned half_y = (unsigned)cv_ceil((r.w - r.y) / 2.0);
-    int q = 0;
-    if ((float)((unsigned)r.x + half_x) <= (float)cand_x(c)) q += 1;
-    if ((float)((unsigned)r.y + half_y) <= (float)cand_y(c)) q += 2;
-    return q;
-}
-
-__device__ __forceinline__ short4 child_rect(const short4 r, int q) {
-    const int half_x = cv_ceil((r.z - r.x) / 2.0), half_y = cv_ceil((r.w - r.y) / 2.0);
-    short4 c;
-    c.x = (q & 1) ? (short)(r.x + half_x) : r.x;
-    c.z = (q & 1) ? r.z : (short)(r.x + half_x);
-    c.y = (q & 2) ? (short)(r.y + half_y) : r.y;
-    c.w = (q & 2) ? r.w : (short)(r.y + half_y);
-    return c;
-}
-
-__device__ void segmented_class_scan(const QtArrays &A, int cur, int n, const QtNodes &N, const uint8_t *sel,
-                                     unsigned short *rank, uint8_t *cls, unsigned short *tot,
-                                     unsigned long long *carry_tail, uint8_t *carry_head) {
-    const int tid = threadIdx.x;
-    const int per = (n + kQtThreads - 1) / kQtThreads;
-    const int i0 = min(n, tid * per), i1 = min(n, i0 + per);
-    const unsigned short *perm = A.perm[cur], *owner = A.owner[cur];
-    unsigned long long acc = 0;
-    bool head = false;
-    int prev_owner = (i0 > 0 && i0 < n) ? owner[i0 - 1] : -1;
-    for (int i = i0; i < i1; ++i) {
-        const int o = owner[i];
-        if (o != prev_owner) {
-            head = true;
-            acc = 0;
-        }
-        prev_owner = o;
-        int q = 0;
-        if (sel[o]) q = classify(N.rect[o], A.cand[perm[i]]);
-        cls[i] = (uint8_t)q;
-        if (sel[o]) acc += 1ull << (16 * q);
-    }
-    carry_tail[tid] = acc;
-    carry_head[tid] = head ? 1 : 0;
-    __syncthreads();
-    if (tid < 32) {
-        constexpr int kPer = kQtThreads / 32;
-        unsigned long long run = 0;
-        bool hf = false;
-        for (int t = tid * kPer; t < (tid + 1) * kPer; ++t) {
-            const bool h = carry_head[t] != 0;
-            run = h ? carry_tail[t] : run + carry_tail[t];
-            hf = hf || h;
-        }
-        unsigned long long v = run;
-        int f = hf ? 1 : 0;
-#pragma unroll
-        for (int o = 1; o < 32; o <<= 1) {
-            const unsigned long long pv = __shfl_up_sync(0xffffffffu, v, o);
-            const int pf = __shfl_up_sync(0xffffffffu, f, o);
-            if (tid >= o) {
-                if (!f) v += pv;
-                f |= pf;
-            }
-        }
-        unsigned long long carry = __shfl_up_sync(0xffffffffu, v, 1);
-        if (tid == 0) carry = 0;
-        run = carry;
-        for (int t = tid * kPer; t < (tid + 1) * kPer; ++t) {
-            const bool h = carry_head[t] != 0;
-            const unsigned long long tail = carry_tail[t];
-            carry_tail[t] = run;
-            run = h ? tail : run + tail;
-        }
-    }
-    __syncthreads();
-    acc = carry_tail[tid];
-    prev_owner = (i0 > 0 && i0 < n) ? owner[i0 - 1] : -1;
-    for (int i = i0; i < i1; ++i) {
-        const int o = owner[i];
-        if (o != prev_owner) acc = 0;
-        prev_owner = o;
-        const int q = cls[i];
-        if (sel[o]) {
-            rank[i] = (unsigned short)((acc >> (16 * q)) & 0xffff);
-            acc += 1ull << (16 * q);
-        }
-        const bool last = (i + 1 == n) || (owner[i + 1] != o);
-        if (last && sel[o]) {
-            tot[o * 4 + 0] = (unsigned short)(acc & 0xffff);
-            tot[o * 4 + 1] = (unsigned short)((acc >> 16) & 0xffff);
-            tot[o * 4 + 2] = (unsigned short)((acc >> 32) & 0xffff);
-            tot[o * 4 + 3] = (unsigned short)((acc >> 48) & 0xffff);
-        }
-    }
-    __syncthreads();
-}
-
-template <int NC>
-struct QtSharedT {
-    short4 rect[2][NC];
-    unsigned short start[2][NC];
-    unsigned short cnt[2][NC];
-    uint8_t leaf[2][NC];
-    uint8_t sel[NC];
-    unsigned short tot[NC * 4];
-    int newpos[NC];
-    int scan[NC];
-    unsigned short pool[2][NC];
-    unsigned short pool_sorted[NC];
-    unsigned long long carry_tail[kQtThreads];
-    uint8_t carry_head[kQtThreads];
-    int warp_tmp[17];
-    int misc[8];
-};
-
-template <int NC>
-__device__ int apply_division(QtSharedT<NC> &S, QtArrays &A, int &cur, int n_cand, int &cur_n, int len, int num_proc,
-                              const unsigned short *proc_list ,
-                              unsigned short *rank, uint8_t *cls, int *pool_len_out, int pool_dst) {
-    const int tid = threadIdx.x;
-    const int nxt_n = cur_n ^ 1;
-    for (int k = tid; k < num_proc; k += kQtThreads) {
-        const int p = proc_list[k];
-        const unsigned short *t = S.tot + p * 4;
-        S.scan[k] = (t[0] > 0) + (t[1] > 0) + (t[2] > 0) + (t[3] > 0);
-    }
-    __syncthreads();
-    const int total_children = block_scan_array(S.scan, num_proc, S.warp_tmp);
-    for (int p = tid; p < len; p += kQtThreads) S.newpos[p] = S.sel[p] ? 0 : 1;
-    __syncthreads();
-    {
-    }
-    const int kept = block_scan_array(S.newpos, len, S.warp_tmp);
-    const int new_len = total_children + kept;
-    for (int p = tid; p < len; p += kQtThreads) {
-        if (!S.sel[p]) {
-            const int pos = total_children + S.newpos[p];
-            S.rect[nxt_n][pos] = S.rect[cur_n][p];
-            S.start[nxt_n][pos] = S.start[cur_n][p];
-            S.cnt[nxt_n][pos] = S.cnt[cur_n][p];
-            S.leaf[nxt_n][pos] = S.leaf[cur_n][p];
-            S.newpos[p] = pos;
-        }
-    }
-    __syncthreads();
-    for (int k = tid; k < num_proc; k += kQtThreads) {
-        const int p = proc_list[k];
-        const unsigned short *t = S.tot + p * 4;
-        const int nch = (t[0] > 0) + (t[1] > 0) + (t[2] > 0) + (t[3] > 0);
-        const int base = total_children - S.scan[k] - nch;
-        const short4 r = S.rect[cur_n][p];
-        int o = S.start[cur_n][p];
-        int rnk = 0;
-        for (int q = 0; q < 4; ++q) {
-            if (t[q] == 0) continue;
-            const int pos = base + (nch - 1 - rnk);
-            S.rect[nxt_n][pos] = child_rect(r, q);
-            S.start[nxt_n][pos] = (unsigned short)o;
-            S.cnt[nxt_n][pos] = t[q];
-            S.leaf[nxt_n][pos] = 0;
-            o += t[q];
-            ++rnk;
-        }
-        S.newpos[p] = base;
-    }
-    __syncthreads();
-    {
-        const unsigned short *perm = A.perm[cur], *owner = A.owner[cur];
-        unsigned short *perm2 = A.perm[cur ^ 1], *owner2 = A.owner[cur ^ 1];
-        for (int i = tid; i < n_cand; i += kQtThreads) {
-            const int o = owner[i];
-            if (S.sel[o]) {
-                const unsigned short *t = S.tot + o * 4;
-                const int q = cls[i];
-                int off = 0, rnk = 0;
-                for (int c = 0; c < q; ++c) {
-                    off += t[c];
-                    rnk += (t[c] > 0);
-                }
-                const int nch = (t[0] > 0) + (t[1] > 0) + (t[2] > 0) + (t[3] > 0);
-                const int dst = S.start[cur_n][o] + off + rank[i];
-                perm2[dst] = perm[i];
-                owner2[dst] = (unsigned short)(S.newpos[o] + (nch - 1 - rnk));
-            } else {
-                perm2[i] = perm[i];
-                owner2[i] = (unsigned short)S.newpos[o];
-            }
-        }
-    }
-    __syncthreads();
-    for (int k = tid; k < num_proc; k += kQtThreads) {
-        const unsigned short *t = S.tot + proc_list[k] * 4;
-        S.scan[k] = (t[0] > 1) + (t[1] > 1) + (t[2] > 1) + (t[3] > 1);
-    }
-    __syncthreads();
-    const int pool_len = block_scan_array(S.scan, num_proc, S.warp_tmp);
-    for (int k = tid; k < num_proc; k += kQtThreads) {
-        const int p = proc_list[k];
-        const unsigned short *t = S.tot + p * 4;
-        const int nch = (t[0] > 0) + (t[1] > 0) + (t[2] > 0) + (t[3] > 0);
-        int w = S.scan[k], rnk = 0;
-        for (int q = 0; q < 4; ++q) {
-            if (t[q] == 0) continue;
-            if (t[q] > 1) S.pool[pool_dst][w++] = (unsigned short)(S.newpos[p] + (nch - 1 - rnk));
-            ++rnk;
-        }
-    }
-    __syncthreads();
-    *pool_len_out = pool_len;
-    cur ^= 1;
-    cur_n = nxt_n;
-    return new_len;
-}
-
-template <int NC, int CC, int kMinBlocks>
-__global__ void __launch_bounds__(kQtThreads, kMinBlocks) quadtree_kernel(OrbDev P) {
-    extern __shared__ __align__(16) uint8_t qsmem[];
-    using QtShared = QtSharedT<NC>;
-    constexpr int kQtSmemCands = CC;
-    QtShared &S = *reinterpret_cast<QtShared *>(qsmem);
-    const int l = blockIdx.x, b = blockIdx.y, tid = threadIdx.x;
-    const LevelInfo &LV = P.lv[l];
-    int *lvl_cnt = P.lvl_cnt + (size_t)b * P.num_levels + l;
-    LevelKp *out = P.lvl_kp + (size_t)b * P.total_slots + LV.slot_base;
-
-    const int *cc = P.cell_cnt + (size_t)b * P.num_cells + LV.cell_base;
-    for (int c = tid; c < LV.num_cells; c += kQtThreads) S.scan[c] = cc[c];
-    __syncthreads();
-    int n = block_scan_array(S.scan, LV.num_cells, S.warp_tmp);
-    if (n == 0) {
-        if (tid == 0) *lvl_cnt = 0;
-        return;
-    }
-    if (n > 65535) {
-        n = 65535;
-        if (tid == 0) P.status[b] = 1;
-    }
-    QtArrays A;
-    unsigned short *rank;
-    uint8_t *cls;
-    {
-        uint8_t *base;
-        if (n <= kQtSmemCands) {
-            base = qsmem + ((sizeof(QtShared) + 15) & ~(size_t)15);
-        } else {
-            base = P.qt_scratch + ((size_t)b * P.num_levels + l) * P.qt_scratch_per_job;
-        }
-        const size_t cap = n <= kQtSmemCands ? kQtSmemCands : 65536;
-        A.cand = reinterpret_cast<uint32_t *>(base);
-        base += cap * 4;
-        A.perm[0] = reinterpret_cast<unsigned short *>(base);
-        base += cap * 2;
-        A.perm[1] = reinterpret_cast<unsigned short *>(base);
-        base += cap * 2;
-        A.owner[0] = reinterpret_cast<unsigned short *>(base);
-        base += cap * 2;
-        A.owner[1] = reinterpret_cast<unsigned short *>(base);
-        base += cap * 2;
-        rank = reinterpret_cast<unsigned short *>(base);
-        base += cap * 2;
-        cls = base;
-    }
-    {
-        const uint32_t *cb = P.cell_buf + ((size_t)b * P.num_cells + LV.cell_base) * kCellCap;
-        for (int c = 0; c < LV.num_cells; ++c) {
-            const int o = S.scan[c], k = cc[c];
-            for (int i = tid; i < k; i += kQtThreads)
-                if (o + i < n) A.cand[o + i] = cb[(size_t)c * kCellCap + i];
-        }
-    }
-    __syncthreads();
-
-    const int min_x = kPatchRadius, max_x = LV.w - kPatchRadius, min_y = kPatchRadius, max_y = LV.h - kPatchRadius;
-    const double ratio = (double)(max_x - min_x) / (max_y - min_y);
-    int gx, gy;
-    double dx, dy;
-    if (ratio > 1) {
-        gx = (int)round(ratio);
-        gy = 1;
-        dx = (double)(max_x - min_x) / gx;
-        dy = max_y - min_y;
-    } else {
-        gx = 1;
-        gy = (int)round(1 / ratio);
-        dx = max_x - min_y;
-        dy = (double)(max_y - min_y) / gy;
-    }
-    const int g = gx * gy;
-    int cur = 0, cur_n = 0, len = 0;
-    {
-        int *cnts = S.scan;
-        for (int i = tid; i < g; i += kQtThreads) cnts[i] = 0;
-        __syncthreads();
-        for (int i = tid; i < n; i += kQtThreads) {
-            const uint32_t c = A.cand[i];
-            const unsigned ix = (unsigned)((float)cand_x(c) / dx), iy = (unsigned)((float)cand_y(c) / dy);
-            int node = (int)(ix + iy * gx);
-            node = min(node, g - 1);
-            cls[i] = 0;
-            A.owner[0][i] = (unsigned short)node;
-            atomicAdd(&cnts[node], 1);
-        }
-        __syncthreads();
-        if (tid == 0) {
-            int off = 0, pos = 0;
-            for (int i = 0; i < g; ++i) {
-                const int c = cnts[i];
-                S.newpos[i] = off;
-                if (c > 0) {
-                    const int ix = i % gx, iy = i / gx;
-                    short4 r;
-                    r.x = (short)(int)(dx * ix);
-                    r.y = (short)(int)(dy * iy);
-                    r.z = (short)(int)(dx * (ix + 1));
-                    r.w = (short)(int)(dy * (iy + 1));
-                    S.rect[0][pos] = r;
-                    S.start[0][pos] = (unsigned short)off;
-                    S.cnt[0][pos] = (unsigned short)c;
-                    S.leaf[0][pos] = (c == 1);
-                    S.tot[i] = (unsigned short)pos;
-                    ++pos;
-                }
-                off += c;
-            }
-            S.misc[0] = pos;
-        }
-        __syncthreads();
-        len = S.misc[0];
-        for (int node = 0; node < g; ++node) {
-            if (cnts[node] == 0) continue;
-            const int per = (n + kQtThreads - 1) / kQtThreads;
-            const int i0 = min(n, tid * per), i1 = min(n, i0 + per);
-            int c = 0;
-            for (int i = i0; i < i1; ++i) c += (A.owner[0][i] == node);
-            int tot;
-            int run = block_exclusive_scan(c, S.warp_tmp, &tot);
-            const int base = S.newpos[node];
-            const unsigned short lp = S.tot[node];
-            for (int i = i0; i < i1; ++i)
-                if (A.owner[0][i] == node) {
-                    A.perm[1][base + run] = (unsigned short)i;
-                    A.owner[1][base + run] = lp;
-                    ++run;
-                }
-            __syncthreads();
-        }
-        cur = 1;
-    }
-    const int budget = LV.budget;
-    int pool_len = 0, pool_cur = 0;
-    bool filled = false;
-    unsigned short *proc_list = S.pool_sorted;
-
-    while (true) {
-        const int prev = len;
-        for (int p = tid; p < len; p += kQtThreads) S.sel[p] = S.leaf[cur_n][p] ? 0 : 1;
-        __syncthreads();
-        for (int p = tid; p < len; p += kQtThreads) S.scan[p] = S.sel[p];
-        __syncthreads();
-        const int num_proc = block_scan_array(S.scan, len, S.warp_tmp);
-        for (int p = tid; p < len; p += kQtThreads)
-            if (S.sel[p]) proc_list[S.scan[p]] = (unsigned short)p;
-        __syncthreads();
-        segmented_class_scan(A, cur, n, QtNodes{S.rect[cur_n], S.start[cur_n], S.cnt[cur_n], S.leaf[cur_n]}, S.sel,
-                             rank, cls, S.tot, S.carry_tail, S.carry_head);
-        len = apply_division(S, A, cur, n, cur_n, len, num_proc, proc_list, rank, cls, &pool_len, pool_cur);
-        if (budget <= len || len == prev) {
-            filled = true;
-            break;
-        }
-        if (budget < len + pool_len) break;
-    }
-    while (!filled) {
-        const int prev = len;
-        const unsigned short *pool = S.pool[pool_cur];
-        for (int p = tid; p < len; p += kQtThreads) S.sel[p] = 0;
-        __syncthreads();
-        for (int k = tid; k < pool_len; k += kQtThreads) S.sel[pool[k]] = 1;
-        __syncthreads();
-        segmented_class_scan(A, cur, n, QtNodes{S.rect[cur_n], S.start[cur_n], S.cnt[cur_n], S.leaf[cur_n]}, S.sel,
-                             rank, cls, S.tot, S.carry_tail, S.carry_head);
-        for (int k = tid; k < pool_len; k += kQtThreads) {
-            const int ck = S.cnt[cur_n][pool[k]];
-            int r = 0;
-            for (int j = 0; j < pool_len; ++j) {
-                const int cj = S.cnt[cur_n][pool[j]];
-                r += (cj > ck) || (cj == ck && j > k);
-            }
-            proc_list[r] = pool[k];
-        }
-        __syncthreads();
-        for (int k = tid; k < pool_len; k += kQtThreads) {
-            const unsigned short *t = S.tot + proc_list[k] * 4;
-            S.scan[k] = (t[0] > 0) + (t[1] > 0) + (t[2] > 0) + (t[3] > 0) - 1;
-        }
-        if (tid == 0) {
-            S.misc[1] = pool_len;
-            S.misc[2] = 0;
-        }
-        __syncthreads();
-        block_scan_array(S.scan, pool_len, S.warp_tmp);
-        for (int k = tid; k < pool_len; k += kQtThreads) {
-            const unsigned short *t = S.tot + proc_list[k] * 4;
-            const int inc = (t[0] > 0) + (t[1] > 0) + (t[2] > 0) + (t[3] > 0) - 1;
-            if (prev + S.scan[k] + inc >= budget) {
-                atomicMin(&S.misc[1], k + 1);
-                S.misc[2] = 1;
-            }
-        }
-        __syncthreads();
-        const int num_proc = S.misc[1];
-        const bool reached = S.misc[2] != 0;
-        __syncthreads();
-        for (int k = num_proc + tid; k < pool_len; k += kQtThreads) S.sel[proc_list[k]] = 0;
-        __syncthreads();
-        len = apply_division(S, A, cur, n, cur_n, len, num_proc, proc_list, rank, cls, &pool_len, pool_cur ^ 1);
-        pool_cur ^= 1;
-        if (reached) filled = true;
-        if (filled || budget <= len || len == prev) break;
-    }
-
-    const int n_out = min(len, LV.slot_cap);
-    if (len > LV.slot_cap && tid == 0) P.status[b] = 3;
-    for (int p = tid; p < n_out; p += kQtThreads) {
-        const int st = S.start[cur_n][p], c = S.cnt[cur_n][p];
-        uint32_t best = A.cand[A.perm[cur][st]];
-        for (int k = 1; k < c; ++k) {
-            const uint32_t v = A.cand[A.perm[cur][st + k]];
-            if (cand_score(v) > cand_score(best)) best = v;
-        }
-        LevelKp kp;
-        kp.x = (short)(cand_x(best) + kPatchRadius);
-        kp.y = (short)(cand_y(best) + kPatchRadius);
-        kp.response = cand_score(best);
-        out[p] = kp;
-    }
-    if (tid == 0) *lvl_cnt = n_out;
-}
-
 constexpr int kDescWarps = 4;
 constexpr int kDescRun = 8;
 constexpr int kDescMinBlocks = 5;
@@ -1343,6 +834,29 @@
 }
 
 using namespace plp;
+
+constexpr auto kQtSmall = quadtree_kernel<kNodeCapSmall, kCandCapSmall, kQtThreadsSmall, kQtMinBlocksSmall>;
+constexpr auto kQtLarge = quadtree_kernel<kNodeCap, kCandCapLarge, kQtThreadsLarge, kQtMinBlocksLarge>;
+static_assert(kQtMaxLevels >= kMaxLevels, "the quadtree job holds every pyramid level");
+
+static QtJob qt_job(const OrbDev &D) {
+    QtJob J;
+    J.num_levels = D.num_levels;
+    J.num_cells = D.num_cells;
+    J.total_slots = D.total_slots;
+    for (int l = 0; l < D.num_levels; ++l) {
+        const LevelInfo &V = D.lv[l];
+        J.lv[l] = QtLevel{V.w, V.h, V.cell_base, V.num_cells, V.budget, V.slot_base, V.slot_cap};
+    }
+    J.cell_buf = D.cell_buf;
+    J.cell_cnt = D.cell_cnt;
+    J.lvl_kp = D.lvl_kp;
+    J.lvl_cnt = D.lvl_cnt;
+    J.scratch = D.qt_scratch;
+    J.scratch_per_job = D.qt_scratch_per_job;
+    J.status = D.status;
+    return J;
+}
 
 struct plp_orb {
     plp_ctx *ctx = nullptr;
@@ -1525,7 +1039,7 @@
             ++v0;
         }
     }
-    int qt_max_slots = 0;
+    int qt_max_slots = 0, qt_max_cells = 0;
     size_t pyr_bytes = 0, blur_bytes = 0;
     int slot_base = 0, cell_base = 0;
     plp_status st = PLP_OK;
@@ -1600,6 +1114,11 @@
             }
         }
         cell_base += V.num_cells;
+        qt_max_cells = std::max(qt_max_cells, V.num_cells);
+    }
+    if (st == PLP_OK && qt_max_cells + 1 > 2 * (qt_max_slots <= kNodeCapSmall ? kNodeCapSmall : kNodeCap)) {
+        set_error("orb: a pyramid level of %d FAST cells exceeds the quadtree's cell capacity", qt_max_cells);
+        st = PLP_ERR_CAPACITY;
     }
     if (st != PLP_OK) {
         delete o;
@@ -1643,7 +1162,7 @@
     ORB_ALLOC(o->d_cell_cnt, B * (size_t)D.num_cells * sizeof(int));
     ORB_ALLOC(o->d_lvl_kp, B * (size_t)D.total_slots * sizeof(LevelKp));
     ORB_ALLOC(o->d_lvl_cnt, B * L * sizeof(int));
-    D.qt_scratch_per_job = (size_t)65536 * (4 + 2 * 5 + 1) + 256;
+    D.qt_scratch_per_job = qt_scratch_bytes_per_job();
     ORB_ALLOC(o->d_qt_scratch, B * L * D.qt_scratch_per_job);
     ORB_ALLOC(o->d_status, B * sizeof(int));
     ORB_ALLOC(o->d_kp, B * (size_t)D.out_cap * sizeof(plp_keypoint));
@@ -1668,11 +1187,11 @@
     o->qt_small = qt_max_slots <= kNodeCapSmall;
     plp_status so;
     if (o->qt_small) {
-        o->qt_smem = ((sizeof(QtSharedT<kNodeCapSmall>) + 15) & ~(size_t)15) + (size_t)kCandCapSmall * (4 + 2 * 5 + 1) + 64;
-        so = ensure_smem_optin((const void *)quadtree_kernel<kNodeCapSmall, kCandCapSmall, 2>, o->qt_smem, "quadtree_kernel<small>");
+        o->qt_smem = qt_smem_bytes<kNodeCapSmall, kCandCapSmall, kQtThreadsSmall>();
+        so = ensure_smem_optin((const void *)kQtSmall, o->qt_smem, "quadtree_kernel<small>");
     } else {
-        o->qt_smem = ((sizeof(QtSharedT<kNodeCap>) + 15) & ~(size_t)15) + (size_t)kCandCapLarge * (4 + 2 * 5 + 1) + 64;
-        so = ensure_smem_optin((const void *)quadtree_kernel<kNodeCap, kCandCapLarge, 1>, o->qt_smem, "quadtree_kernel<large>");
+        o->qt_smem = qt_smem_bytes<kNodeCap, kCandCapLarge, kQtThreadsLarge>();
+        so = ensure_smem_optin((const void *)kQtLarge, o->qt_smem, "quadtree_kernel<large>");
     }
     if (so != PLP_OK) {
         plp_orb_destroy(o);
@@ -1740,10 +1259,11 @@
     {
         dim3 grid(D.num_levels, batch);
         if (ctx->timing) plp::timing_begin(ctx, o->qt_small ? "quadtree_kernel<1024>" : "quadtree_kernel<2048>");
+        const QtJob J = qt_job(D);
         if (o->qt_small)
-            quadtree_kernel<kNodeCapSmall, kCandCapSmall, 2><<<grid, kQtThreads, o->qt_smem, ctx->stream>>>(D);
+            kQtSmall<<<grid, kQtThreadsSmall, o->qt_smem, ctx->stream>>>(J);
         else
-            quadtree_kernel<kNodeCap, kCandCapLarge, 1><<<grid, kQtThreads, o->qt_smem, ctx->stream>>>(D);
+            kQtLarge<<<grid, kQtThreadsLarge, o->qt_smem, ctx->stream>>>(J);
         if (ctx->timing) plp::timing_end(ctx);
         ctx->launches++;
     }
diff --git a/structure-plp-slam_b200/csrc/quadtree_kernels.cuh b/structure-plp-slam_b200/csrc/quadtree_kernels.cuh
--- /dev/null
+++ b/structure-plp-slam_b200/csrc/quadtree_kernels.cuh
@@ -0,0 +1,566 @@
+#pragma once
+#include <math.h>
+#include <stddef.h>
+#include <stdint.h>
+
+#include "devmath.cuh"
+
+namespace plp {
+
+namespace {
+
+constexpr int kPatchRadius = 19;
+constexpr int kCellCap = 1024;
+constexpr int kQtMaxLevels = 16;
+
+constexpr int kNodeCapSmall = 1024, kCandCapSmall = 2048, kQtThreadsSmall = 256, kQtMinBlocksSmall = 3;
+constexpr int kNodeCap = 2048, kCandCapLarge = 8192, kQtThreadsLarge = 512, kQtMinBlocksLarge = 1;
+constexpr int kQtScratchCands = 65536;
+constexpr int kQtCandBytes = 4 + 2 * 5 + 1;
+
+struct LevelKp {
+    short x, y;
+    int response;
+};
+
+struct QtLevel {
+    int w, h;
+    int cell_base, num_cells;
+    int budget;
+    int slot_base, slot_cap;
+};
+
+struct QtJob {
+    int num_levels;
+    int num_cells;
+    int total_slots;
+    QtLevel lv[kQtMaxLevels];
+    const uint32_t *cell_buf;
+    const int *cell_cnt;
+    LevelKp *lvl_kp;
+    int *lvl_cnt;
+    uint8_t *scratch;
+    size_t scratch_per_job;
+    int *status;
+};
+
+__host__ __device__ constexpr size_t qt_scratch_bytes_per_job() { return (size_t)kQtScratchCands * kQtCandBytes + 256; }
+
+struct QtArrays {
+    uint32_t *cand;
+    unsigned short *perm[2];
+    unsigned short *owner[2];
+};
+
+__device__ __forceinline__ int cand_x(uint32_t c) { return (int)(c & 0x7ff); }
+__device__ __forceinline__ int cand_y(uint32_t c) { return (int)((c >> 11) & 0x3ff); }
+__device__ __forceinline__ int cand_score(uint32_t c) { return (int)(c >> 21); }
+
+template <int T>
+__device__ __forceinline__ void qt_chunk(int n, int &i0, int &i1) {
+    const int per = (n + T - 1) / T;
+    i0 = min(n, (int)threadIdx.x * per);
+    i1 = min(n, i0 + per);
+}
+
+template <int T, class V>
+__device__ __forceinline__ V qt_block_scan(V v, V *wbuf, V *total) {
+    const int lane = threadIdx.x & 31, warp = threadIdx.x >> 5;
+    V incl = v;
+#pragma unroll
+    for (int o = 1; o < 32; o <<= 1) {
+        const V t = __shfl_up_sync(0xffffffffu, incl, o);
+        if (lane >= o) incl += t;
+    }
+    if (lane == 31) wbuf[warp] = incl;
+    __syncthreads();
+    V pre = 0, tot = 0;
+#pragma unroll
+    for (int w = 0; w < T / 32; ++w) {
+        const V s = wbuf[w];
+        if (w < warp) pre += s;
+        tot += s;
+    }
+    *total = tot;
+    return pre + incl - v;
+}
+
+__device__ __forceinline__ int classify(const short4 r, uint32_t c) {
+    const unsigned half_x = (unsigned)cv_ceil((r.z - r.x) / 2.0);
+    const unsigned half_y = (unsigned)cv_ceil((r.w - r.y) / 2.0);
+    int q = 0;
+    if ((float)((unsigned)r.x + half_x) <= (float)cand_x(c)) q += 1;
+    if ((float)((unsigned)r.y + half_y) <= (float)cand_y(c)) q += 2;
+    return q;
+}
+
+__device__ __forceinline__ short4 child_rect(const short4 r, int q) {
+    const int half_x = cv_ceil((r.z - r.x) / 2.0), half_y = cv_ceil((r.w - r.y) / 2.0);
+    short4 c;
+    c.x = (q & 1) ? (short)(r.x + half_x) : r.x;
+    c.z = (q & 1) ? r.z : (short)(r.x + half_x);
+    c.y = (q & 2) ? (short)(r.y + half_y) : r.y;
+    c.w = (q & 2) ? r.w : (short)(r.y + half_y);
+    return c;
+}
+
+template <int NC, int T>
+struct QtSharedT {
+    short4 rect[2][NC];
+    unsigned short start[2][NC];
+    unsigned short cnt[2][NC];
+    uint8_t leaf[2][NC];
+    uint8_t sel[NC];
+    unsigned short newpos[NC];
+    unsigned short pool[NC];
+    unsigned short proc[NC];
+    union {
+        unsigned short tot[NC * 4];
+        int cell_pre[NC * 2];
+    } u;
+    unsigned long long wsum[2][T / 32];
+    unsigned long long seg_tail[T / 32];
+    int seg_head[T / 32];
+    int misc[4];
+};
+
+struct QtScan {
+    unsigned long long *buf;
+    int stride, next;
+    __device__ unsigned long long *get() {
+        unsigned long long *b = buf + next * stride;
+        next ^= 1;
+        return b;
+    }
+};
+
+template <int T>
+__device__ __forceinline__ int qt_block_scan_int(int v, QtScan &sc, int *total) {
+    unsigned long long t;
+    const unsigned long long pre = qt_block_scan<T, unsigned long long>((unsigned long long)v, sc.get(), &t);
+    *total = (int)t;
+    return (int)pre;
+}
+
+template <int NC, int T>
+__device__ __forceinline__ void segmented_class_scan(QtSharedT<NC, T> &S, const QtArrays &A, int cur, int n, int cur_n,
+                                     unsigned short *rank, uint8_t *cls) {
+    const int lane = threadIdx.x & 31, warp = threadIdx.x >> 5;
+    int i0, i1;
+    qt_chunk<T>(n, i0, i1);
+    const unsigned short *perm = A.perm[cur], *owner = A.owner[cur];
+    const short4 *rect = S.rect[cur_n];
+    unsigned long long acc = 0;
+    int head = 0;
+    int prev_owner = (i0 > 0 && i0 < n) ? owner[i0 - 1] : -1;
+    for (int i = i0; i < i1; ++i) {
+        const int o = owner[i];
+        if (o != prev_owner) {
+            head = 1;
+            acc = 0;
+        }
+        prev_owner = o;
+        int q = 0;
+        if (S.sel[o]) {
+            q = classify(rect[o], A.cand[perm[i]]);
+            acc += 1ull << (16 * q);
+        }
+        cls[i] = (uint8_t)q;
+    }
+    unsigned long long v = acc;
+    int f = head;
+#pragma unroll
+    for (int o = 1; o < 32; o <<= 1) {
+        const unsigned long long pv = __shfl_up_sync(0xffffffffu, v, o);
+        const int pf = __shfl_up_sync(0xffffffffu, f, o);
+        if (lane >= o) {
+            if (!f) v += pv;
+            f |= pf;
+        }
+    }
+    if (lane == 31) {
+        S.seg_tail[warp] = v;
+        S.seg_head[warp] = f;
+    }
+    unsigned long long ev = __shfl_up_sync(0xffffffffu, v, 1);
+    int ef = __shfl_up_sync(0xffffffffu, f, 1);
+    if (lane == 0) {
+        ev = 0;
+        ef = 0;
+    }
+    __syncthreads();
+    unsigned long long carry = 0;
+    for (int w = 0; w < warp; ++w) carry = S.seg_head[w] ? S.seg_tail[w] : carry + S.seg_tail[w];
+    acc = ef ? ev : carry + ev;
+    prev_owner = (i0 > 0 && i0 < n) ? owner[i0 - 1] : -1;
+    for (int i = i0; i < i1; ++i) {
+        const int o = owner[i];
+        if (o != prev_owner) acc = 0;
+        prev_owner = o;
+        if (S.sel[o]) {
+            const int q = cls[i];
+            rank[i] = (unsigned short)((acc >> (16 * q)) & 0xffff);
+            acc += 1ull << (16 * q);
+            const bool last = (i + 1 == n) || (owner[i + 1] != o);
+            if (last) {
+                unsigned short *t = S.u.tot + o * 4;
+                t[0] = (unsigned short)(acc & 0xffff);
+                t[1] = (unsigned short)((acc >> 16) & 0xffff);
+                t[2] = (unsigned short)((acc >> 32) & 0xffff);
+                t[3] = (unsigned short)((acc >> 48) & 0xffff);
+            }
+        }
+    }
+    __syncthreads();
+}
+
+__device__ __forceinline__ unsigned long long qt_child_counts(const unsigned short *t) {
+    const int nch = (t[0] > 0) + (t[1] > 0) + (t[2] > 0) + (t[3] > 0);
+    const int npool = (t[0] > 1) + (t[1] > 1) + (t[2] > 1) + (t[3] > 1);
+    return (unsigned long long)nch | ((unsigned long long)npool << 16);
+}
+
+template <int NC, int T>
+__device__ __forceinline__ int divide_nodes(QtSharedT<NC, T> &S, QtArrays &A, int &cur, int n_cand, int &cur_n, int len,
+                            const unsigned short *proc, int num_proc, const unsigned short *rank, const uint8_t *cls,
+                            int *pool_len_out, QtScan &sc) {
+    const int tid = threadIdx.x;
+    const int nxt_n = cur_n ^ 1;
+    int p0, p1, k0, k1;
+    qt_chunk<T>(len, p0, p1);
+    if (proc) {
+        qt_chunk<T>(num_proc, k0, k1);
+    } else {
+        k0 = p0;
+        k1 = p1;
+    }
+    unsigned long long local = 0;
+    for (int k = k0; k < k1; ++k) {
+        const int p = proc ? proc[k] : k;
+        if (proc || S.sel[p]) local += qt_child_counts(S.u.tot + p * 4);
+    }
+    for (int p = p0; p < p1; ++p)
+        if (!S.sel[p]) local += 1ull << 32;
+    unsigned long long total;
+    const unsigned long long pre = qt_block_scan<T, unsigned long long>(local, sc.get(), &total);
+    const int total_children = (int)(total & 0xffff), pool_len = (int)((total >> 16) & 0xffff);
+    const int new_len = total_children + (int)(total >> 32);
+    int cpre = (int)(pre & 0xffff), ppre = (int)((pre >> 16) & 0xffff), kpre = (int)(pre >> 32);
+    for (int k = k0; k < k1; ++k) {
+        const int p = proc ? proc[k] : k;
+        if (!proc && !S.sel[p]) continue;
+        const unsigned short *t = S.u.tot + p * 4;
+        const int nch = (t[0] > 0) + (t[1] > 0) + (t[2] > 0) + (t[3] > 0);
+        const int base = total_children - cpre - nch;
+        const short4 r = S.rect[cur_n][p];
+        int o = S.start[cur_n][p];
+        int rnk = 0;
+        for (int q = 0; q < 4; ++q) {
+            if (t[q] == 0) continue;
+            const int pos = base + (nch - 1 - rnk);
+            S.rect[nxt_n][pos] = child_rect(r, q);
+            S.start[nxt_n][pos] = (unsigned short)o;
+            S.cnt[nxt_n][pos] = t[q];
+            S.leaf[nxt_n][pos] = 0;
+            if (t[q] > 1) S.pool[ppre++] = (unsigned short)pos;
+            o += t[q];
+            ++rnk;
+        }
+        S.newpos[p] = (unsigned short)base;
+        cpre += nch;
+    }
+    for (int p = p0; p < p1; ++p) {
+        if (S.sel[p]) continue;
+        const int pos = total_children + kpre++;
+        S.rect[nxt_n][pos] = S.rect[cur_n][p];
+        S.start[nxt_n][pos] = S.start[cur_n][p];
+        S.cnt[nxt_n][pos] = S.cnt[cur_n][p];
+        S.leaf[nxt_n][pos] = S.leaf[cur_n][p];
+        S.newpos[p] = (unsigned short)pos;
+    }
+    __syncthreads();
+    {
+        const unsigned short *perm = A.perm[cur], *owner = A.owner[cur];
+        unsigned short *perm2 = A.perm[cur ^ 1], *owner2 = A.owner[cur ^ 1];
+        for (int i = tid; i < n_cand; i += T) {
+            const int o = owner[i];
+            if (S.sel[o]) {
+                const unsigned short *t = S.u.tot + o * 4;
+                const int q = cls[i];
+                int off = 0, rnk = 0;
+                for (int c = 0; c < q; ++c) {
+                    off += t[c];
+                    rnk += (t[c] > 0);
+                }
+                const int nch = (t[0] > 0) + (t[1] > 0) + (t[2] > 0) + (t[3] > 0);
+                const int dst = S.start[cur_n][o] + off + rank[i];
+                perm2[dst] = perm[i];
+                owner2[dst] = (unsigned short)(S.newpos[o] + (nch - 1 - rnk));
+            } else {
+                perm2[i] = perm[i];
+                owner2[i] = S.newpos[o];
+            }
+        }
+    }
+    __syncthreads();
+    *pool_len_out = pool_len;
+    cur ^= 1;
+    cur_n = nxt_n;
+    return new_len;
+}
+
+template <int NC, int CC, int T, int kMinBlocks>
+__global__ void __launch_bounds__(T, kMinBlocks) quadtree_kernel(QtJob P) {
+    PLP_DYNAMIC_SMEM(qsmem);
+    using QtShared = QtSharedT<NC, T>;
+    QtShared &S = *reinterpret_cast<QtShared *>(qsmem);
+    const int l = blockIdx.x, b = blockIdx.y, tid = threadIdx.x;
+    const QtLevel &LV = P.lv[l];
+    int *lvl_cnt = P.lvl_cnt + (size_t)b * P.num_levels + l;
+    LevelKp *out = P.lvl_kp + (size_t)b * P.total_slots + LV.slot_base;
+    QtScan sc{S.wsum[0], T / 32, 0};
+
+    const int *cc = P.cell_cnt + (size_t)b * P.num_cells + LV.cell_base;
+    const int num_cells = LV.num_cells;
+    int *cpre = S.u.cell_pre;
+    int n;
+    {
+        int c0, c1;
+        qt_chunk<T>(num_cells, c0, c1);
+        int sum = 0;
+        for (int c = c0; c < c1; ++c) {
+            cpre[c] = cc[c];
+            sum += cpre[c];
+        }
+        int run = qt_block_scan_int<T>(sum, sc, &n);
+        for (int c = c0; c < c1; ++c) {
+            const int k = cpre[c];
+            cpre[c] = run;
+            run += k;
+        }
+        if (tid == 0) cpre[num_cells] = n;
+        __syncthreads();
+    }
+    if (n == 0) {
+        if (tid == 0) *lvl_cnt = 0;
+        return;
+    }
+    if (n > 65535) {
+        n = 65535;
+        if (tid == 0) P.status[b] = 1;
+    }
+    QtArrays A;
+    unsigned short *rank;
+    uint8_t *cls;
+    {
+        uint8_t *base;
+        if (n <= CC) {
+            base = qsmem + ((sizeof(QtShared) + 15) & ~(size_t)15);
+        } else {
+            base = P.scratch + ((size_t)b * P.num_levels + l) * P.scratch_per_job;
+        }
+        const size_t cap = n <= CC ? CC : kQtScratchCands;
+        A.cand = reinterpret_cast<uint32_t *>(base);
+        base += cap * 4;
+        A.perm[0] = reinterpret_cast<unsigned short *>(base);
+        base += cap * 2;
+        A.perm[1] = reinterpret_cast<unsigned short *>(base);
+        base += cap * 2;
+        A.owner[0] = reinterpret_cast<unsigned short *>(base);
+        base += cap * 2;
+        A.owner[1] = reinterpret_cast<unsigned short *>(base);
+        base += cap * 2;
+        rank = reinterpret_cast<unsigned short *>(base);
+        base += cap * 2;
+        cls = base;
+    }
+    {
+        constexpr int kBatch = 4;
+        const uint32_t *cb = P.cell_buf + ((size_t)b * P.num_cells + LV.cell_base) * kCellCap;
+        for (int i0 = tid; i0 < n; i0 += kBatch * T) {
+            uint32_t v[kBatch];
+#pragma unroll
+            for (int j = 0; j < kBatch; ++j) {
+                const int i = i0 + j * T;
+                if (i < n) {
+                    int lo = 0, hi = num_cells;
+                    while (hi - lo > 1) {
+                        const int mid = (lo + hi) >> 1;
+                        if (cpre[mid] <= i) lo = mid;
+                        else hi = mid;
+                    }
+                    v[j] = __ldg(cb + (size_t)lo * kCellCap + (i - cpre[lo]));
+                }
+            }
+#pragma unroll
+            for (int j = 0; j < kBatch; ++j)
+                if (i0 + j * T < n) A.cand[i0 + j * T] = v[j];
+        }
+    }
+    __syncthreads();
+
+    const int min_x = kPatchRadius, max_x = LV.w - kPatchRadius, min_y = kPatchRadius, max_y = LV.h - kPatchRadius;
+    const double ratio = (double)(max_x - min_x) / (max_y - min_y);
+    int gx, gy;
+    double dx, dy;
+    if (ratio > 1) {
+        gx = (int)round(ratio);
+        gy = 1;
+        dx = (double)(max_x - min_x) / gx;
+        dy = max_y - min_y;
+    } else {
+        gx = 1;
+        gy = (int)round(1 / ratio);
+        dx = max_x - min_y;
+        dy = (double)(max_y - min_y) / gy;
+    }
+    const int g = gx * gy;
+    int cur = 0, cur_n = 0, len = 0;
+    {
+        int *cnts = S.u.cell_pre;
+        for (int i = tid; i < g; i += T) cnts[i] = 0;
+        __syncthreads();
+        for (int i = tid; i < n; i += T) {
+            const uint32_t c = A.cand[i];
+            const unsigned ix = (unsigned)((float)cand_x(c) / dx), iy = (unsigned)((float)cand_y(c) / dy);
+            int node = (int)(ix + iy * gx);
+            node = min(node, g - 1);
+            A.owner[0][i] = (unsigned short)node;
+            atomicAdd(&cnts[node], 1);
+        }
+        __syncthreads();
+        if (tid == 0) {
+            int off = 0, pos = 0;
+            for (int i = 0; i < g; ++i) {
+                const int c = cnts[i];
+                S.newpos[i] = (unsigned short)off;
+                if (c > 0) {
+                    const int ix = i % gx, iy = i / gx;
+                    short4 r;
+                    r.x = (short)(int)(dx * ix);
+                    r.y = (short)(int)(dy * iy);
+                    r.z = (short)(int)(dx * (ix + 1));
+                    r.w = (short)(int)(dy * (iy + 1));
+                    S.rect[0][pos] = r;
+                    S.start[0][pos] = (unsigned short)off;
+                    S.cnt[0][pos] = (unsigned short)c;
+                    S.leaf[0][pos] = (c == 1);
+                    S.proc[i] = (unsigned short)pos;
+                    ++pos;
+                }
+                off += c;
+            }
+            S.misc[0] = pos;
+        }
+        __syncthreads();
+        len = S.misc[0];
+        int i0, i1;
+        qt_chunk<T>(n, i0, i1);
+        for (int node = 0; node < g; ++node) {
+            if (cnts[node] == 0) continue;
+            int c = 0;
+            for (int i = i0; i < i1; ++i) c += (A.owner[0][i] == node);
+            int tot;
+            int run = qt_block_scan_int<T>(c, sc, &tot);
+            const int base = S.newpos[node];
+            const unsigned short lp = S.proc[node];
+            for (int i = i0; i < i1; ++i)
+                if (A.owner[0][i] == node) {
+                    A.perm[1][base + run] = (unsigned short)i;
+                    A.owner[1][base + run] = lp;
+                    ++run;
+                }
+        }
+        __syncthreads();
+        cur = 1;
+    }
+    const int budget = LV.budget;
+    int pool_len = 0;
+    bool filled = false;
+
+    while (true) {
+        const int prev = len;
+        for (int p = tid; p < len; p += T) S.sel[p] = S.leaf[cur_n][p] ? 0 : 1;
+        __syncthreads();
+        segmented_class_scan(S, A, cur, n, cur_n, rank, cls);
+        len = divide_nodes(S, A, cur, n, cur_n, len, (const unsigned short *)nullptr, 0, rank, cls, &pool_len, sc);
+        if (budget <= len || len == prev) {
+            filled = true;
+            break;
+        }
+        if (budget < len + pool_len) break;
+    }
+    while (!filled) {
+        const int prev = len;
+        for (int p = tid; p < len; p += T) S.sel[p] = 0;
+        if (tid == 0) S.misc[1] = pool_len + 1;
+        __syncthreads();
+        for (int k = tid; k < pool_len; k += T) {
+            S.sel[S.pool[k]] = 1;
+            S.newpos[k] = S.cnt[cur_n][S.pool[k]];
+        }
+        __syncthreads();
+        segmented_class_scan(S, A, cur, n, cur_n, rank, cls);
+        for (int k = tid; k < pool_len; k += T) {
+            const int ck = S.newpos[k];
+            int r = 0;
+            for (int j = 0; j < pool_len; ++j) {
+                const int cj = S.newpos[j];
+                r += (cj > ck) || (cj == ck && j > k);
+            }
+            S.proc[r] = S.pool[k];
+        }
+        __syncthreads();
+        int num_proc;
+        bool reached;
+        {
+            int k0, k1;
+            qt_chunk<T>(pool_len, k0, k1);
+            int sum = 0;
+            for (int k = k0; k < k1; ++k) sum += (int)(qt_child_counts(S.u.tot + S.proc[k] * 4) & 0xffff) - 1;
+            int tot;
+            int run = prev + qt_block_scan_int<T>(sum, sc, &tot);
+            for (int k = k0; k < k1; ++k) {
+                run += (int)(qt_child_counts(S.u.tot + S.proc[k] * 4) & 0xffff) - 1;
+                if (run >= budget) {
+                    atomicMin(&S.misc[1], k + 1);
+                    break;
+                }
+            }
+            __syncthreads();
+            reached = S.misc[1] <= pool_len;
+            num_proc = reached ? S.misc[1] : pool_len;
+        }
+        for (int k = num_proc + tid; k < pool_len; k += T) S.sel[S.proc[k]] = 0;
+        __syncthreads();
+        len = divide_nodes(S, A, cur, n, cur_n, len, S.proc, num_proc, rank, cls, &pool_len, sc);
+        if (reached) filled = true;
+        if (filled || budget <= len || len == prev) break;
+    }
+
+    const int n_out = min(len, LV.slot_cap);
+    if (len > LV.slot_cap && tid == 0) P.status[b] = 3;
+    for (int p = tid; p < n_out; p += T) {
+        const int st = S.start[cur_n][p], c = S.cnt[cur_n][p];
+        uint32_t best = A.cand[A.perm[cur][st]];
+        for (int k = 1; k < c; ++k) {
+            const uint32_t v = A.cand[A.perm[cur][st + k]];
+            if (cand_score(v) > cand_score(best)) best = v;
+        }
+        LevelKp kp;
+        kp.x = (short)(cand_x(best) + kPatchRadius);
+        kp.y = (short)(cand_y(best) + kPatchRadius);
+        kp.response = cand_score(best);
+        out[p] = kp;
+    }
+    if (tid == 0) *lvl_cnt = n_out;
+}
+
+template <int NC, int CC, int T>
+__host__ __device__ constexpr size_t qt_smem_bytes() {
+    return ((sizeof(QtSharedT<NC, T>) + 15) & ~(size_t)15) + (size_t)CC * kQtCandBytes + 64;
+}
+
+}
+
+}
```

New measurement: 87840 (median of 6 runs). 1.05x the previous value.
